# mnlevy1981/MOM6

Measured on AMD Instinct MI355X. Metric: simulated-years/day (SYPD) of the split-RK2 dynamical core + tracer advection + ALE remap, higher is better.
Workload: dtype f64

## Files before the change

### include/mom6hip.h

```cpp
#ifndef MOM6HIP_H
#define MOM6HIP_H

#include <stdint.h>

#ifdef __cplusplus
extern "C" {
#endif

#define MOM6HIP_MEM_HOST   0
#define MOM6HIP_MEM_DEVICE 1

#define MOM6HIP_ADV_PLM    0
#define MOM6HIP_ADV_PPM_H3 1
#define MOM6HIP_ADV_PPM    2

typedef struct mom6hip_grid {
  int32_t isc, iec, jsc, jec;
  int32_t isd, ied, jsd, jed;
  int32_t nk;
  int32_t symmetric;
  int32_t reentrant_x, reentrant_y;
  int32_t first_direction;
  int32_t tripolar_n;
  double Angstrom_H;
// ... 338 lines not shown
#define MOM6HIP_EOS_WRIGHT_REDUCED 5

typedef struct mom6hip_eos {
  int32_t form;
  int32_t reserved;
  double Rho_T0_S0, dRho_dT, dRho_dS;
} mom6hip_eos_t;

typedef struct mom6hip_pressureforce_cs {
  double Rho0;
  double GFS_scale;
  double Z_ref;
  int32_t reconstruct;
  int32_t Recon_Scheme;
  int32_t boundary_extrap;
  int32_t useMassWghtInterp;
  int32_t use_ALE;
  int32_t nkmb;
  double P_Ref;
  const double *Rlay;
  const double *g_prime;
} mom6hip_pressureforce_cs_t;

int mom6hip_pressureforce_fv_bouss(mom6hip_ctx_t *ctx, const mom6hip_pressureforce_cs_t *cs, const mom6hip_eos_t *eos,
                                   const double *h, const double *T, const double *S, const double *p_atm,
                                   double *PFu, double *PFv, double *pbce, double *eta, int32_t memspace);
int mom6hip_pgf_face_launches(mom6hip_ctx_t *ctx, uint64_t *counts);

int mom6hip_pressureforce_fv_nonbouss(mom6hip_ctx_t *ctx, const mom6hip_pressureforce_cs_t *cs, const mom6hip_eos_t *eos,
                                      const double *h, const double *T, const double *S, const double *p_atm, double H_to_RZ,
                                      double *PFu, double *PFv, double *pbce, double *eta, int32_t memspace);

int mom6hip_calculate_density(mom6hip_ctx_t *ctx, const mom6hip_eos_t *eos, const double *T, const double *S,
                              const double *pressure, double *rho, int64_t n, int32_t use_rho_ref, double rho_ref,
                              int32_t memspace);


#define MOM6HIP_BT_HARMONIC     1
#define MOM6HIP_BT_ARITHMETIC   2
#define MOM6HIP_BT_HYBRID       3
#define MOM6HIP_BT_FROM_BT_CONT 4

typedef struct mom6hip_barotropic_cs {
  double dtbt;
  double dtbt_max;
  double dtbt_fraction;
  double bebt;
  double dt_bt_filter;
  double vel_underflow;
  double G_extra;
  double BT_Coriolis_scale;
  double Z_ref;
  double maxCFL_BT_cont;
  double reserved0[6];
  int32_t Sadourny;
  int32_t linearized_BT_PV;
  int32_t strong_drag;
  int32_t visc_rem_u_uh0;
  int32_t adjust_BT_cont;
  int32_t use_wide_halos;
  int32_t hvel_scheme;
  int32_t nstep_last;
  int32_t unsupported[12];
  int32_t bound_BT_corr;
  int32_t BT_project_velocity;
  int32_t Nonlinear_continuity;
  int32_t Nonlin_cont_update_period;
  double *frhatu, *frhatv;
  double *eta_cor;
  double *IDatu, *IDatv;
  double *ubtav, *vbtav;
  double *q_D;
  double *D_u_Cor, *D_v_Cor;
  void *reserved2[6];
} mom6hip_barotropic_cs_t;

int mom6hip_barotropic_init(mom6hip_ctx_t *ctx, mom6hip_barotropic_cs_t *cs, int32_t memspace);

int mom6hip_btcalc(mom6hip_ctx_t *ctx, mom6hip_barotropic_cs_t *cs, const double *h, const double *h_u,
                   const double *h_v, int32_t may_use_default, int32_t memspace);
int mom6hip_btcalc_obc(mom6hip_ctx_t *ctx, mom6hip_barotropic_cs_t *cs, const double *h, const double *h_u, const double *h_v,
                       int32_t may_use_default, const struct mom6hip_obc *obc, int32_t memspace);

int mom6hip_bt_mass_source(mom6hip_ctx_t *ctx, mom6hip_barotropic_cs_t *cs, const double *h, const double *eta,
                           int32_t set_cor, int32_t memspace);

int mom6hip_set_dtbt_eta(mom6hip_ctx_t *ctx, mom6hip_barotropic_cs_t *cs, const double *eta, const double *pbce,
                         const mom6hip_bt_cont_t *BT_cont, double gtot_est, double SSH_add, int32_t memspace);
int mom6hip_set_dtbt(mom6hip_ctx_t *ctx, mom6hip_barotropic_cs_t *cs, const double *pbce,
                     const mom6hip_bt_cont_t *BT_cont, double gtot_est, double SSH_add, int32_t memspace);

int mom6hip_bt_graph_stats(mom6hip_ctx_t *ctx, int64_t *captures, int64_t *launches);
int mom6hip_bt_graph_nodes(mom6hip_ctx_t *ctx, int64_t *nodes);

int mom6hip_btstep(mom6hip_ctx_t *ctx, mom6hip_barotropic_cs_t *cs, const double *U_in, const double *V_in,
                   const double *eta_in, double dt, const double *bc_accel_u, const double *bc_accel_v,
                   const double *taux, const double *tauy, double RZ_to_H, const double *pbce,
                   const double *eta_PF_in, const double *U_Cor, const double *V_Cor, double *accel_layer_u,
                   double *accel_layer_v, double *eta_out, double *uhbtav, double *vhbtav,
                   const double *visc_rem_u, const double *visc_rem_v, const mom6hip_bt_cont_t *BT_cont,
                   const double *eta_PF_start, const double *taux_bot, const double *tauy_bot, const double *uh0,
                   const double *vh0, const double *u_uh0, const double *v_vh0, double *etaav, int32_t memspace);
int mom6hip_btstep_obc(mom6hip_ctx_t *ctx, mom6hip_barotropic_cs_t *cs, const double *U_in, const double *V_in, const double *eta_in,
                       double dt, const double *bc_accel_u, const double *bc_accel_v, const double *taux, const double *tauy,
                       double RZ_to_H, const double *pbce, const double *eta_PF_in, const double *U_Cor, const double *V_Cor,
                       double *accel_layer_u, double *accel_layer_v, double *eta_out, double *uhbtav, double *vhbtav,
                       const double *visc_rem_u, const double *visc_rem_v, const mom6hip_bt_cont_t *BT_cont, const double *eta_PF_start,
                       const double *taux_bot, const double *tauy_bot, const double *uh0, const double *vh0, const double *u_uh0,
                       const double *v_vh0, double *etaav, const struct mom6hip_obc *obc, int32_t memspace);


typedef struct mom6hip_vertvisc_cs {
  double Hmix;
  double Hmix_stress;
  double Kvml_invZ2;
  double Kv;
  double Hbbl;
  double Kv_extra_bbl;
  double harm_BL_val;
  double maxvel;
  double CFL_trunc;
  double vel_underflow;
  double H_to_RZ;
  double vonKar;
  int32_t dynamic_viscous_ML;
  int32_t nkml;
  double reserved0[3];
  int32_t bottomdraglaw;
  int32_t harmonic_visc;
  int32_t direct_stress;
  int32_t CFL_based_trunc;
  int32_t answer_date;
  int32_t unsupported[7];
  int64_t ntrunc;
  double *a_u, *a_v, *h_u, *h_v;
  void *reserved1[4];
} mom6hip_vertvisc_cs_t;

typedef struct mom6hip_vertvisc_type {
  const double *Kv_bbl_u, *Kv_bbl_v;
  const double *bbl_thick_u, *bbl_thick_v;
  const double *Ray_u, *Ray_v;
  const double *Kv_shear;
  const double *Kv_shear_Bu;
  const double *nkml_visc_u, *nkml_visc_v;
  const double *ustar;
  const void *reserved[1];
} mom6hip_vertvisc_type_t;

int mom6hip_vertvisc_coef(mom6hip_ctx_t *ctx, mom6hip_vertvisc_cs_t *cs, const double *u, const double *v, const double *h,
                          const double *dz, const mom6hip_vertvisc_type_t *visc, double dt, int32_t memspace);

int mom6hip_vertvisc(mom6hip_ctx_t *ctx, mom6hip_vertvisc_cs_t *cs, double *u, double *v, const double *h, const double *taux,
                     const double *tauy, const mom6hip_vertvisc_type_t *visc, double dt, double *taux_bot, double *tauy_bot,
                     int32_t memspace);

int mom6hip_vertvisc_coef_obc(mom6hip_ctx_t *ctx, mom6hip_vertvisc_cs_t *cs, const double *u, const double *v, const double *h,
                              const double *dz, const mom6hip_vertvisc_type_t *visc, double dt, const struct mom6hip_obc *obc,
                              int32_t memspace);
int mom6hip_vertvisc_obc(mom6hip_ctx_t *ctx, mom6hip_vertvisc_cs_t *cs, double *u, double *v, const double *h, const double *taux,
                         const double *tauy, const mom6hip_vertvisc_type_t *visc, double dt, double *taux_bot, double *tauy_bot,
                         const struct mom6hip_obc *obc, int32_t memspace);

int mom6hip_vertvisc_and_remnant(mom6hip_ctx_t *ctx, mom6hip_vertvisc_cs_t *cs, double *u, double *v, const double *h,
                                 const double *taux, const double *tauy, const mom6hip_vertvisc_type_t *visc, double dt,
                                 double *taux_bot, double *tauy_bot, double *visc_rem_u, double *visc_rem_v, int32_t memspace);
// ... 310 lines not shown
```

### mom6_amd/_lib.py

```python
import ctypes as C
import os

from . import _abi

_HERE = os.path.dirname(os.path.abspath(__file__))
LIB_PATH = os.environ.get("MOM6HIP_LIB_PATH") or os.path.join(_HERE, "libmom6hip.so")
_LIB = None
_dp = C.POINTER(C.c_double)

EXPORTS = (
    "mom6hip_init", "mom6hip_last_error", "mom6hip_grid_create", "mom6hip_grid_destroy",
    "mom6hip_sync", "mom6hip_malloc", "mom6hip_free", "mom6hip_sync_to_device",
    "mom6hip_sync_to_host", "mom6hip_halo_update", "mom6hip_advect_tracer", "mom6hip_set_timing",
    "mom6hip_advect_get_timing", "mom6hip_ale_remap_tracers", "mom6hip_ale_plm_edge_values", "mom6hip_coradcalc", "mom6hip_continuity", "mom6hip_pressureforce_fv_bouss", "mom6hip_pressureforce_fv_nonbouss", "mom6hip_pgf_face_launches", "mom6hip_calculate_density", "mom6hip_set_domain_callbacks",
    "mom6hip_barotropic_init", "mom6hip_btcalc", "mom6hip_bt_mass_source", "mom6hip_set_dtbt", "mom6hip_memset_zero", "mom6hip_transfer_stats", "mom6hip_debug_poison_passes", "mom6hip_tracer_hordiff_varmix", "mom6hip_tracer_hordiff_neutral", "mom6hip_tracer_hordiff_epipycnal", "mom6hip_continuity_obc", "mom6hip_coradcalc_obc", "mom6hip_vertvisc_coef_obc", "mom6hip_update_segment_tracer_reservoirs", "mom6hip_advect_tracer_obc", "mom6hip_btstep_obc", "mom6hip_horizontal_viscosity_obc", "mom6hip_set_viscous_bbl_obc", "mom6hip_btcalc_obc", "mom6hip_vertvisc_obc", "mom6hip_radiation_open_bdry_conds", "mom6hip_open_boundary_zero_normal_flow", "mom6hip_overlap_stats", "mom6hip_thickness_diffuse", "mom6hip_mixedlayer_restrat", "mom6hip_mixedlayer_restrat_mu", "mom6hip_start_group_pass", "mom6hip_complete_group_pass", "mom6hip_set_dtbt_eta", "mom6hip_btstep",
    "mom6hip_dyn_split_rk2_init", "mom6hip_step_dyn_split_rk2", "mom6hip_dyn_split_rk2b_init", "mom6hip_step_dyn_split_rk2b",
    "mom6hip_ale_regrid", "mom6hip_ale_remap_set_h_vel", "mom6hip_ale_remap_set_h_vel_via_dz", "mom6hip_ale_remap_velocities", "mom6hip_halo_pack", "mom6hip_set_min_callback", "mom6hip_kernel_timing", "mom6hip_set_callback_stream_ordered", "mom6hip_bt_graph_stats", "mom6hip_bt_graph_nodes",
    "mom6hip_vertvisc_coef", "mom6hip_vertvisc", "mom6hip_vertvisc_remnant", "mom6hip_vertvisc_ntrunc", "mom6hip_vertvisc_and_remnant", "mom6hip_vertvisc_step",
    "mom6hip_hor_visc_init", "mom6hip_horizontal_viscosity", "mom6hip_set_viscous_bbl", "mom6hip_set_viscous_ml",
    "mom6hip_chksum", "mom6hip_reproducing_sum", "mom6hip_write_energy_sums", "mom6hip_depth_list_create", "mom6hip_write_energy_ape", "mom6hip_host_register", "mom6hip_host_unregister", "mom6hip_stage_to_host",
    "mom6hip_stage_query", "mom6hip_stage_wait", "mom6hip_stream_bandwidth", "mom6hip_graph_node_floor", "mom6hip_tracer_hordiff", "mom6hip_tracer_hordiff_hbd", "mom6hip_rccl_get_unique_id", "mom6hip_domain_init_rccl", "mom6hip_domain_exchange_timing",
)


class Mom6HipError(RuntimeError):
    pass


def lib():
    global _LIB
    if _LIB is None:
        if not os.path.exists(LIB_PATH):
            raise Mom6HipError(
                f"{LIB_PATH} not found: build it with `python -c 'import __graft_entry__ as g; g.build()'` "
                "(make -C mom6_amd/csrc). mom6_amd has no CPU fallback.")
        import importlib.util
        if importlib.util.find_spec("torch") is not None:
            import torch
        L = C.CDLL(LIB_PATH)
        L.mom6hip_last_error.restype = C.c_char_p
        L.mom6hip_init.argtypes = [C.c_int]
        L.mom6hip_grid_create.argtypes = [C.POINTER(_abi.GridStruct), C.c_void_p, C.POINTER(C.c_void_p)]
        L.mom6hip_grid_destroy.argtypes = [C.c_void_p]
        L.mom6hip_sync.argtypes = [C.c_void_p]
        L.mom6hip_malloc.argtypes = [C.POINTER(C.c_void_p), C.c_uint64]
        L.mom6hip_free.argtypes = [C.c_void_p]
        L.mom6hip_sync_to_device.argtypes = [C.c_void_p, C.c_void_p, C.c_void_p, C.c_uint64]
        L.mom6hip_sync_to_host.argtypes = [C.c_void_p, C.c_void_p, C.c_void_p, C.c_uint64]
        L.mom6hip_halo_update.argtypes = [C.c_void_p, C.POINTER(C.c_void_p), C.POINTER(C.c_int32),
                                          C.POINTER(C.c_int32), C.c_int32]
        L.mom6hip_advect_tracer.argtypes = [
            C.c_void_p, C.c_void_p, C.c_void_p, C.c_void_p, C.c_double,
            C.POINTER(_abi.TracerAdvectCS), C.POINTER(C.c_void_p), _dp, C.c_int32, C.c_int32,
            C.c_void_p, C.c_int32, C.c_int32, C.c_void_p, C.c_void_p, C.c_int32,
            C.POINTER(_abi.AdvectStats)]
        L.mom6hip_set_timing.argtypes = [C.c_void_p, C.c_int32]
        L.mom6hip_advect_get_timing.argtypes = [C.c_void_p, C.POINTER(_abi.AdvectTiming)]
        L.mom6hip_ale_remap_tracers.argtypes = [C.c_void_p, C.POINTER(_abi.RemappingCS), C.c_void_p, C.c_void_p,
                                                C.POINTER(C.c_void_p), _dp, C.c_int32, C.c_int32]
        L.mom6hip_coradcalc.argtypes = [C.c_void_p, C.POINTER(_abi.CoriolisAdvCS)] + [C.c_void_p] * 7 + [C.c_int32]
        L.mom6hip_continuity.argtypes = ([C.c_void_p, C.POINTER(_abi.ContinuityCS)] + [C.c_void_p] * 6 + [C.c_double]
                                         + [C.c_void_p] * 6 + [C.POINTER(_abi.BTCont)] + [C.c_void_p] * 2 + [C.c_int32])
        L.mom6hip_pressureforce_fv_bouss.argtypes = ([C.c_void_p, C.POINTER(_abi.PressureForceCS), C.POINTER(_abi.EOS)]
                                                     + [C.c_void_p] * 8 + [C.c_int32])
        L.mom6hip_pressureforce_fv_nonbouss.argtypes = ([C.c_void_p, C.POINTER(_abi.PressureForceCS), C.POINTER(_abi.EOS)]
                                                        + [C.c_void_p] * 4 + [C.c_double] + [C.c_void_p] * 4 + [C.c_int32])
        L.mom6hip_calculate_density.argtypes = ([C.c_void_p, C.POINTER(_abi.EOS)] + [C.c_void_p] * 4
                                                + [C.c_int64, C.c_int32, C.c_double, C.c_int32])
        L.mom6hip_set_domain_callbacks.argtypes = [C.c_void_p, C.c_void_p, C.c_void_p, C.c_void_p]
        L.mom6hip_kernel_timing.argtypes = [C.c_void_p, C.c_int32, C.POINTER(C.c_double), C.POINTER(C.c_int64)]
        L.mom6hip_bt_graph_stats.argtypes = [C.c_void_p, C.POINTER(C.c_int64), C.POINTER(C.c_int64)]
        L.mom6hip_set_callback_stream_ordered.argtypes = [C.c_void_p, C.c_int32]
        L.mom6hip_set_min_callback.argtypes = [C.c_void_p, C.c_void_p, C.c_void_p]
        L.mom6hip_halo_pack.argtypes = [C.c_void_p, C.POINTER(C.c_void_p), C.POINTER(C.c_int32), C.POINTER(C.c_int32),
                                        C.POINTER(C.c_int32), C.c_int32, C.c_int32, C.c_int32, C.c_void_p, C.c_int32,
                                        C.POINTER(C.c_int64)]
        for n in ("grid", "tracer_advect_cs", "advect_stats", "advect_timing"):
            getattr(L, f"mom6hip_abi_sizeof_{n}").restype = C.c_uint64
        L.mom6hip_abi_offsetof_grid_mask2dT.restype = C.c_uint64
        _LIB = L
    return _LIB


def check(rc, what):
    if rc != 0:
        msg = lib().mom6hip_last_error().decode("utf-8", "replace")
        raise Mom6HipError(f"{what}: {msg} (rc={rc})")
```

### mom6_amd/barotropic.py

```python
from __future__ import annotations

import ctypes as C

import numpy as np
import torch

from . import _abi
from ._lib import Mom6HipError, check, lib
from .continuity import BT_cont_type
from .tracer_advect import DeviceGrid, _ptr_space

_DEFAULTS = dict(dtbt_fraction=0.98, bebt=0.1, dt_bt_filter=-0.25, vel_underflow=0.0, G_extra=0.0, BT_Coriolis_scale=1.0,
                 Z_ref=0.0, Sadourny=True, linearized_BT_PV=True, strong_drag=False, visc_rem_u_uh0=False,
                 adjust_BT_cont=False, use_wide_halos=True)
_PARAM_NAMES = {"BEBT": "bebt", "DT_BT_FILTER": "dt_bt_filter", "VEL_UNDERFLOW": "vel_underflow", "G_BT_EXTRA": "G_extra",
                "BT_CORIOLIS_SCALE": "BT_Coriolis_scale", "REFERENCE_HEIGHT": "Z_ref", "SADOURNY": "Sadourny",
                "LINEARIZED_BT_CORIOLIS": "linearized_BT_PV", "BT_STRONG_DRAG": "strong_drag",
                "BT_USE_VISC_REM_U_UH0": "visc_rem_u_uh0", "ADJUST_BT_CONT": "adjust_BT_cont",
                "BT_USE_WIDE_HALOS": "use_wide_halos"}


class barotropic_CS:

    def __init__(self, G, device="cuda", DTBT=-0.98, BT_THICK_SCHEME=None, USE_BT_CONT_TYPE=True, **params):
        g = G.grid if isinstance(G, DeviceGrid) else G
        d = dict(_DEFAULTS)
        unsupported = [0] * 12
        bound = bool(params.pop("BOUND_BT_CORRECTION", False))
        cont_bounds = bool(params.pop("BT_CONT_CORR_BOUNDS", True))
        maxcfl = float(params.pop("MAXCFL_BT_CONT", 0.25))
        project = bool(params.pop("BT_PROJECT_VELOCITY", False))
        nonlin = bool(params.pop("NONLINEAR_BT_CONTINUITY", False))
        nonlin_period = int(params.pop("NONLIN_BT_CONT_UPDATE_PERIOD", 1))
        if bound and not (USE_BT_CONT_TYPE and cont_bounds):
            unsupported[3] = 1
        for k, v in params.items():
            if k in _PARAM_NAMES:
                d[_PARAM_NAMES[k]] = v
            elif k in d:
                d[k] = v
            elif k in _abi.BT_UNSUPPORTED:
                unsupported[_abi.BT_UNSUPPORTED.index(k)] = int(bool(v))
            else:
                raise Mom6HipError(f"barotropic_init: unknown parameter {k}")
        st = _abi.BarotropicCS()
        for k, v in d.items():
            setattr(st, k, float(v) if isinstance(getattr(st, k), float) else int(bool(v)))
        if BT_THICK_SCHEME is None:
            BT_THICK_SCHEME = "FROM_BT_CONT" if USE_BT_CONT_TYPE else "HYBRID"
        if BT_THICK_SCHEME == "FROM_BT_CONT" and not USE_BT_CONT_TYPE:
            raise Mom6HipError("barotropic_init: BT_THICK_SCHEME FROM_BT_CONT can only be used if USE_BT_CONT_TYPE is defined.")
        st.hvel_scheme = _abi.BT_THICK_SCHEMES[BT_THICK_SCHEME]
        st.bound_BT_corr, st.maxCFL_BT_cont = int(bound), maxcfl
        st.BT_project_velocity = int(project)
        st.Nonlinear_continuity, st.Nonlin_cont_update_period = int(nonlin), nonlin_period
        for q in range(12):
            st.unsupported[q] = unsupported[q]
        self.dtbt_input = float(DTBT)
        st.dtbt_fraction = 0.98 if DTBT >= 0.0 else -float(DTBT)
        st.dtbt = float(DTBT) if DTBT > 0.0 else 0.0
        self.grid, self.device, self.st = g, device, st
        self.arrays = {}
        for n, pos, nd in _abi.BT_CS_ARRAYS:
            shp = g.shape3(pos) if nd == 3 else g.shape2(pos)
            a = np.zeros(shp) if device == "cpu" else torch.zeros(shp, dtype=torch.float64, device=device)
            self.arrays[n] = a
            setattr(st, n, _ptr_space(a)[0])
        self.space = _ptr_space(self.arrays["frhatu"])[1]
        self.module_is_initialized = False

    def __getattr__(self, n):
        a = self.__dict__.get("arrays", {})
        if n in a:
            return a[n]
        st = self.__dict__.get("st")
        if st is not None and hasattr(st, n):
            return getattr(st, n)
        raise AttributeError(n)


def _P(spaces, a):
    if a is None:
        return None
    p, s = _ptr_space(a)
    spaces.add(s)
    return C.c_void_p(p)


def _one_space(spaces, CS, who):
    spaces.add(CS.space)
    if len(spaces) != 1:
        raise Mom6HipError(f"{who}: all fields and the control structure must be in the same memory space")
    return spaces.pop()


def _setup():
    L = lib()
    if not getattr(L, "_bt_ready", False):
        cs = C.POINTER(_abi.BarotropicCS)
        L.mom6hip_barotropic_init.argtypes = [C.c_void_p, cs, C.c_int32]
        L.mom6hip_btcalc.argtypes = [C.c_void_p, cs, C.c_void_p, C.c_void_p, C.c_void_p, C.c_int32, C.c_int32]
        L.mom6hip_btcalc_obc.argtypes = [C.c_void_p, cs, C.c_void_p, C.c_void_p, C.c_void_p, C.c_int32, C.POINTER(_abi.Obc), C.c_int32]
        L.mom6hip_bt_mass_source.argtypes = [C.c_void_p, cs, C.c_void_p, C.c_void_p, C.c_int32, C.c_int32]
        L.mom6hip_set_dtbt.argtypes = [C.c_void_p, cs, C.c_void_p, C.POINTER(_abi.BTCont), C.c_double, C.c_double, C.c_int32]
        L.mom6hip_set_dtbt_eta.argtypes = [C.c_void_p, cs, C.c_void_p, C.c_void_p, C.POINTER(_abi.BTCont), C.c_double, C.c_double, C.c_int32]
        L.mom6hip_btstep.argtypes = ([C.c_void_p, cs] + [C.c_void_p] * 3 + [C.c_double] + [C.c_void_p] * 4 + [C.c_double]
                                     + [C.c_void_p] * 11 + [C.POINTER(_abi.BTCont)] + [C.c_void_p] * 8 + [C.c_int32])
        L.mom6hip_btstep_obc.argtypes = ([C.c_void_p, cs] + [C.c_void_p] * 3 + [C.c_double] + [C.c_void_p] * 4 + [C.c_double]
                                         + [C.c_void_p] * 11 + [C.POINTER(_abi.BTCont)] + [C.c_void_p] * 8 + [C.POINTER(_abi.Obc), C.c_int32])
        L._bt_ready = True
    return L


def barotropic_init(G: DeviceGrid, device="cuda", gtot_estimate=None, SSH_extra=None, **params) -> barotropic_CS:
    CS = barotropic_CS(G, device=device, **params)
    L = _setup()
    check(L.mom6hip_barotropic_init(G.handle, C.byref(CS.st), CS.space), "barotropic_init")
    CS.module_is_initialized = True
    g = CS.grid
    if gtot_estimate is None:
        gtot_estimate = g.H_to_Z * g.g_Earth
    if SSH_extra is None:
        SSH_extra = min(10.0, 0.05 * float(np.max(g.bathyT)))
    dtbt_in = CS.dtbt_input
    set_dtbt(G, CS, gtot_est=gtot_estimate, SSH_add=SSH_extra)
    if dtbt_in > 0.0:
        CS.st.dtbt = dtbt_in
    return CS


def btcalc(h, G: DeviceGrid, CS: barotropic_CS, h_u=None, h_v=None, may_use_default=False, OBC=None):
    if not CS.module_is_initialized:
        raise Mom6HipError("btcalc: Module MOM_barotropic must be initialized before it is used.")
    sp = set()
    args = [_P(sp, h), _P(sp, h_u), _P(sp, h_v)]
    if OBC is not None:
        obc = OBC.struct(lambda a: (0, None))
        check(_setup().mom6hip_btcalc_obc(G.handle, C.byref(CS.st), *args, int(bool(may_use_default)), C.byref(obc),
                                          _one_space(sp, CS, "btcalc")), "btcalc")
        return
    check(_setup().mom6hip_btcalc(G.handle, C.byref(CS.st), *args, int(bool(may_use_default)), _one_space(sp, CS, "btcalc")), "btcalc")


def bt_mass_source(h, eta, set_cor, G: DeviceGrid, CS: barotropic_CS):
    if not CS.module_is_initialized:
        raise Mom6HipError("bt_mass_source: Module MOM_barotropic must be initialized before it is used.")
    sp = set()
    args = [_P(sp, h), _P(sp, eta)]
    check(_setup().mom6hip_bt_mass_source(G.handle, C.byref(CS.st), *args, int(bool(set_cor)), _one_space(sp, CS, "bt_mass_source")),
          "bt_mass_source")


def set_dtbt(G: DeviceGrid, CS: barotropic_CS, eta=None, pbce=None, BT_cont: BT_cont_type | None = None, gtot_est=None,
             SSH_add=0.0):
    if not CS.module_is_initialized:
        raise Mom6HipError("set_dtbt: Module MOM_barotropic must be initialized before it is used.")
    if pbce is None and gtot_est is None:
        raise Mom6HipError("set_dtbt: Either pbce or gtot_est must be present.")
    sp = set()
    p = _P(sp, pbce)
    pe = _P(sp, eta)
    bt = None if BT_cont is None else BT_cont.struct(sp)
    check(_setup().mom6hip_set_dtbt_eta(G.handle, C.byref(CS.st), pe, p, None if bt is None else C.byref(bt),
                                    0.0 if gtot_est is None else float(gtot_est), float(SSH_add), _one_space(sp, CS, "set_dtbt")),
          "set_dtbt")
    return CS.st.dtbt_max


def btstep(U_in, V_in, eta_in, dt, bc_accel_u, bc_accel_v, forces, pbce, eta_PF_in, U_Cor, V_Cor, accel_layer_u,
           accel_layer_v, eta_out, uhbtav, vhbtav, G: DeviceGrid, CS: barotropic_CS, visc_rem_u, visc_rem_v, SpV_avg=None,
           ADp=None, OBC=None, BT_cont: BT_cont_type | None = None, eta_PF_start=None, taux_bot=None, tauy_bot=None, uh0=None,
           vh0=None, u_uh0=None, v_vh0=None, etaav=None):
    if not CS.module_is_initialized:
        raise Mom6HipError("btstep: Module MOM_barotropic must be initialized before it is used.")
    if (uh0 is not None) and (vh0 is None or u_uh0 is None or v_vh0 is None):
        raise Mom6HipError("btstep: vh0, u_uh0, and v_vh0 must be associated if uh0 is used.")
    g = CS.grid
    taux, tauy = forces
    sp = set()
    P = lambda a: _P(sp, a)
    a1 = [P(U_in), P(V_in), P(eta_in)]
    a2 = [P(bc_accel_u), P(bc_accel_v), P(taux), P(tauy)]
    a3 = [P(x) for x in (pbce, eta_PF_in, U_Cor, V_Cor, accel_layer_u, accel_layer_v, eta_out, uhbtav, vhbtav, visc_rem_u, visc_rem_v)]
    bt = None if BT_cont is None else BT_cont.struct(sp)
    a4 = [P(x) for x in (eta_PF_start, taux_bot, tauy_bot, uh0, vh0, u_uh0, v_vh0, etaav)]
    RZ_to_H = g.Z_to_H / g.Rho0
    space = _one_space(sp, CS, "btstep")
    if OBC is not None:
        from .open_boundary import _seg_to_ptr
        obc = OBC.struct(_seg_to_ptr(space))
        check(_setup().mom6hip_btstep_obc(G.handle, C.byref(CS.st), *a1, float(dt), *a2, float(RZ_to_H), *a3,
                                          None if bt is None else C.byref(bt), *a4, C.byref(obc), space), "btstep")
        return
    check(_setup().mom6hip_btstep(G.handle, C.byref(CS.st), *a1, float(dt), *a2, float(RZ_to_H), *a3,
                                  None if bt is None else C.byref(bt), *a4, space), "btstep")
```

### mom6_amd/csrc/barotropic.hip

```cpp
#include "common.hpp"
#include "cr_math.hpp"

#include <algorithm>
#include <string>
#include <cmath>
#include <cstdlib>
#include <functional>
#include <initializer_list>
#include <utility>

namespace m6 {

}

namespace {

constexpr double SUBROUNDOFF = 1e-30;

using m6::cr::cr_pow;

template <class F> __global__ void __launch_bounds__(256) range2d_kernel(int i0, int i1, int j0, int j1, F f) {
  const int i = i0 + blockIdx.x * 64 + threadIdx.x, j = j0 + blockIdx.y * 4 + threadIdx.y;
  if (i <= i1 && j <= j1) f(i, j);
}
// ... 4 lines not shown
}

struct Btcl { double *FA_EE, *FA_E0, *FA_W0, *FA_WW, *uBT_WW, *uBT_EE, *uh_crvW, *uh_crvE, *uh_WW, *uh_EE; };

__device__ __forceinline__ double find_uhbt(double u, const Btcl &B, long n) {
  if (u == 0.0) return 0.0;
  const double ee = B.uBT_EE[n];
  if (u < ee) return (u - ee) * B.FA_EE[n] + B.uh_EE[n];
  if (u < 0.0) return u * (B.FA_E0[n] + B.uh_crvE[n] * (u * u));
  const double ww = B.uBT_WW[n];
  if (u <= ww) return u * (B.FA_W0[n] + B.uh_crvW[n] * (u * u));
  return (u - ww) * B.FA_WW[n] + B.uh_WW[n];
}

struct Work {
  double *ubt, *bt_rem_u, *BT_force_u, *u_accel_bt, *uhbt, *uhbt0, *uhbtp, *azon, *bzon, *czon, *dzon, *Cor_ref_u,
      *DCor_u, *Datu, *ubt_Cor, *ubt0, *uhbtS, *amer, *bmer, *cmer, *dmer;
  double *vbt, *bt_rem_v, *BT_force_v, *v_accel_bt, *vhbt, *vhbt0, *vhbtp, *Cor_ref_v, *DCor_v, *Datv, *vbt_Cor, *vbt0,
      *vhbtS;
  double *eta, *eta_pred, *eta_sum, *eta_wtd, *eta_PF, *eta_PF_1, *d_eta_PF, *gtot_E, *gtot_W, *gtot_N, *gtot_S,
      *eta_src, *e_anom;
  double *q;
  Btcl BU, BV;
  const int32_t *obc_u, *obc_v;
  double *ob_Cg_u, *ob_dZ_u, *ob_uhbt, *ob_ubt_outer, *ob_SSH_u, *ubt_old, *ubt_first, *ubt_wtd;
  double *ob_Cg_v, *ob_dZ_v, *ob_vhbt, *ob_vbt_outer, *ob_SSH_v, *vbt_old, *vbt_first, *vbt_wtd;
};
enum { OB_SPEC = 1, OB_FLATHER = 2, OB_GRAD = 4, OB_PLUS = 8, OB_MINUS = 16 };

__device__ double uhbt_to_ubt(double uhbt, const Btcl &B, long n) {
  const double tol = 1.0e-10;
  const int max_itt = 20;
  double ubt, ubt_min, ubt_max, uherr_min, uherr_max;
  if (uhbt == 0.0) {
    ubt = 0.0;
  } else if (uhbt < B.uh_EE[n]) {
    ubt = B.uBT_EE[n] + (uhbt - B.uh_EE[n]) / B.FA_EE[n];
  } else if (uhbt < 0.0) {
    ubt_min = B.uBT_EE[n]; uherr_min = B.uh_EE[n] - uhbt;
    ubt_max = 0.0; uherr_max = -uhbt;
    ubt = B.uBT_EE[n] * (uhbt / B.uh_EE[n]);
    for (int itt = 1; itt <= max_itt; itt++) {
      const double uhbt_err = ubt * (B.FA_E0[n] + B.uh_crvE[n] * (ubt * ubt)) - uhbt;
      if (fabs(uhbt_err) < tol * fabs(uhbt)) break;
      if (uhbt_err > 0.0) { ubt_max = ubt; uherr_max = uhbt_err; }
      if (uhbt_err < 0.0) { ubt_min = ubt; uherr_min = uhbt_err; }
      const double derr_du = B.FA_E0[n] + 3.0 * B.uh_crvE[n] * (ubt * ubt);
      if ((uhbt_err >= derr_du * (ubt - ubt_min)) || (-uhbt_err >= derr_du * (ubt_max - ubt)) || (derr_du <= 0.0)) {
        ubt = ubt_max + (ubt_min - ubt_max) * (uherr_max / (uherr_max - uherr_min));
      } else {
        ubt = ubt - uhbt_err / derr_du;
        if (fabs(uhbt_err) < (0.01 * tol) * fabs(ubt_min * derr_du)) break;
      }
    }
  } else if (uhbt <= B.uh_WW[n]) {
    ubt_min = 0.0; uherr_min = -uhbt;
    ubt_max = B.uBT_WW[n]; uherr_max = B.uh_WW[n] - uhbt;
    ubt = B.uBT_WW[n] * (uhbt / B.uh_WW[n]);
    for (int itt = 1; itt <= max_itt; itt++) {
      const double uhbt_err = ubt * (B.FA_W0[n] + B.uh_crvW[n] * (ubt * ubt)) - uhbt;
      if (fabs(uhbt_err) < tol * fabs(uhbt)) break;
      if (uhbt_err > 0.0) { ubt_max = ubt; uherr_max = uhbt_err; }
      if (uhbt_err < 0.0) { ubt_min = ubt; uherr_min = uhbt_err; }
      const double derr_du = B.FA_W0[n] + 3.0 * B.uh_crvW[n] * (ubt * ubt);
      if ((uhbt_err >= derr_du * (ubt - ubt_min)) || (-uhbt_err >= derr_du * (ubt_max - ubt)) || (derr_du <= 0.0)) {
        ubt = ubt_min + (ubt_max - ubt_min) * (-uherr_min / (uherr_max - uherr_min));
      } else {
        ubt = ubt - uhbt_err / derr_du;
        if (fabs(uhbt_err) < (0.01 * tol) * (ubt_max * derr_du)) break;
      }
    }
  } else {
    ubt = B.uBT_WW[n] + (uhbt - B.uh_WW[n]) / B.FA_WW[n];
  }
  return ubt;
}

struct Par {
  double dtbt, Instep, dgeo_de, vel_underflow, trans_wt1, trans_wt2, RZ_to_H;
  int project_velocity;
  int nstep, use_BT_cont, interp_eta_PF, add_uh0, strong_drag, visc_rem_u_uh0, find_etaav, have_bot;
};

template <int DIR>
__global__ void __launch_bounds__(256)
bt_pre_face_kernel(m6::GridDev g, Work w, Par p, const double *__restrict__ frhat, const double *__restrict__ visc_rem,
                   const double *__restrict__ vel_Cor, const double *__restrict__ pbce, const double *__restrict__ uh0,
                   const double *__restrict__ u_uh0, const double *__restrict__ vel_in, const double *__restrict__ bc_accel,
                   const double *__restrict__ tau, const double *__restrict__ tau_bot, const double *__restrict__ IDat) {
  const int i = (DIR ? g.isc : g.isc - 1) + blockIdx.x * 64 + threadIdx.x;
  const int j = (DIR ? g.jsc - 1 : g.jsc) + blockIdx.y * 4 + threadIdx.y;
  if (i > g.iec || j > g.jec) return;
  const long f2 = DIR ? g.v2(i, j) : g.u2(i, j);
  const long fstr = DIR ? (long)g.nih * (g.njh + 1) : (long)(g.nih + 1) * g.njh;
  const long hm = g.h2(i, j), hp = DIR ? g.h2(i, j + 1) : g.h2(i + 1, j), hstr = (long)g.nih * g.njh;
  const double mask = DIR ? g.mask2dCv[f2] : g.mask2dCu[f2];

  double vel_cor = 0.0, gt_m = 0.0, gt_p = 0.0, uhS = 0.0, u0 = 0.0, ub = 0.0, av_rem = 0.0, force;
  if (mask > 0.0) {
    force = tau[f2] * p.RZ_to_H * IDat[f2] * visc_rem[f2];
    if (p.have_bot) force = force - tau_bot[f2] * p.RZ_to_H * IDat[f2];
  } else {
    force = 0.0;
  }
  for (int k = 0; k < g.nk; k++) {
    const long f3 = f2 + fstr * k;
    const double fr = frhat[f3], vr_in = visc_rem[f3];
    double vr = m6::min2(vr_in, 1.);
    vr = m6::max2(vr, 1. - 0.5 * p.Instep / (vr + SUBROUNDOFF));
    vr = m6::max2(vr, 0.);
    const double wt = fr * vr;
    vel_cor = vel_cor + wt * vel_Cor[f3];
    gt_m = gt_m + pbce[hm + hstr * k] * wt;
    gt_p = gt_p + pbce[hp + hstr * k] * wt;
    if (p.add_uh0) {
      uhS = uhS + uh0[f3];
      u0 = u0 + (p.visc_rem_u_uh0 ? wt : fr) * u_uh0[f3];
    }
    ub = ub + wt * vel_in[f3];
    force = force + wt * bc_accel[f3];
    av_rem = av_rem + fr * vr_in;
  }
  if (fabs(ub) < p.vel_underflow) ub = 0.0;
  double rem;
  if (p.strong_drag) {
    rem = mask * ((p.nstep * av_rem) / (1.0 + (p.nstep - 1) * av_rem));
  } else {
    rem = 0.0;
    if (mask * av_rem > 0.0) rem = mask * cr_pow(av_rem, p.Instep);
  }
  if (DIR == 0) {
    w.ubt_Cor[f2] = vel_cor; w.gtot_E[hm] = gt_m; w.gtot_W[hp] = gt_p; w.uhbtS[f2] = uhS; w.ubt0[f2] = u0;
    w.ubt[f2] = ub; w.BT_force_u[f2] = force; w.bt_rem_u[f2] = rem;
  } else {
    w.vbt_Cor[f2] = vel_cor; w.gtot_N[hm] = gt_m; w.gtot_S[hp] = gt_p; w.vhbtS[f2] = uhS; w.vbt0[f2] = u0;
    w.vbt[f2] = ub; w.BT_force_v[f2] = force; w.bt_rem_v[f2] = rem;
  }
}

template <int DIR, int NKMAX>
__global__ void __launch_bounds__(256) __attribute__((amdgpu_waves_per_eu(3, 8)))
btcalc_given_kernel(m6::GridDev g, const double *__restrict__ hw, double *__restrict__ fr, double h_neglect) {
  const int i = (DIR ? g.isc : g.isc - 1) + blockIdx.x * 64 + threadIdx.x;
  const int j = (DIR ? g.jsc - 1 : g.jsc) + blockIdx.y * 4 + threadIdx.y;
  if (i > g.iec || j > g.jec) return;
  const long f2 = DIR ? g.v2(i, j) : g.u2(i, j);
  const long fstr = DIR ? (long)g.nih * (g.njh + 1) : (long)(g.nih + 1) * g.njh;
  const double mask = DIR ? g.mask2dCv[f2] : g.mask2dCu[f2];
  const int nz = g.nk;
  double v[NKMAX];
  const double *__restrict__ src = hw + f2;
#pragma unroll
  for (int k = 0; k < NKMAX; k++) { v[k] = (k < nz) ? *src : 0.0; src += fstr; }
  double tot = v[0];
#pragma unroll
  for (int k = 1; k < NKMAX; k++) if (k < nz) tot = tot + v[k];
  const double Ihat = mask / (tot + h_neglect);
  double *__restrict__ dst = fr + f2;
#pragma unroll
  for (int k = 0; k < NKMAX; k++) { if (k < nz) *dst = v[k] * Ihat; dst += fstr; }
}

template <int DIR>
__global__ void __launch_bounds__(256)
bt_accel_layer_kernel(m6::GridDev g, Work w, const double *__restrict__ pbce, double *__restrict__ accel, double accel_underflow) {
  const int i = (DIR ? g.isc : g.isc - 1) + blockIdx.x * 64 + threadIdx.x;
  const int j = (DIR ? g.jsc - 1 : g.jsc) + blockIdx.y * 4 + threadIdx.y;
  if (i > g.iec || j > g.jec) return;
  const long f2 = DIR ? g.v2(i, j) : g.u2(i, j);
  const long fstr = DIR ? (long)g.nih * (g.njh + 1) : (long)(g.nih + 1) * g.njh;
  const long hm = g.h2(i, j), hp = DIR ? g.h2(i, j + 1) : g.h2(i + 1, j), hstr = (long)g.nih * g.njh;
  const double abt = DIR ? w.v_accel_bt[f2] : w.u_accel_bt[f2];
  const double gp = DIR ? w.gtot_S[hp] : w.gtot_W[hp], gm = DIR ? w.gtot_N[hm] : w.gtot_E[hm];
  const double ep = w.e_anom[hp], em = w.e_anom[hm];
  const double Id = DIR ? g.IdyCv[f2] : g.IdxCu[f2];
  for (int k = 0; k < g.nk; k++) {
    double a = (abt - ((pbce[hp + hstr * k] - gp) * ep - (pbce[hm + hstr * k] - gm) * em) * Id);
    if (fabs(a) < accel_underflow) a = 0.0;
    accel[f2 + fstr * k] = a;
  }
}

__global__ void __launch_bounds__(256)
bt_eta_pred_kernel(m6::GridDev g, Work w, Par p, int i0, int i1, int j0, int j1, double wt_accel2) {
  const int i = i0 + blockIdx.x * 64 + threadIdx.x, j = j0 + blockIdx.y * 4 + threadIdx.y;
  if (i > i1 || j > j1) return;
  const long n = g.h2(i, j);
  double ep;
  if (p.project_velocity) {
    ep = w.eta[n];
  } else {
    ep = (w.eta[n] + w.eta_src[n]) + (p.dtbt * g.IareaT[n]) *
        ((w.uhbtp[g.u2(i - 1, j)] - w.uhbtp[g.u2(i, j)]) + (w.vhbtp[g.v2(i, j - 1)] - w.vhbtp[g.v2(i, j)]));
    w.eta_pred[n] = ep;
  }
  if (p.find_etaav && i >= g.isc && i <= g.iec && j >= g.jsc && j <= g.jec) w.eta_sum[n] = w.eta_sum[n] + wt_accel2 * ep;
}

__global__ void __launch_bounds__(256)
bt_eta_kernel(m6::GridDev g, Work w, Par p, int i0, int i1, int j0, int j1, double wt_eta) {
  const int i = i0 + blockIdx.x * 64 + threadIdx.x, j = j0 + blockIdx.y * 4 + threadIdx.y;
  if (i > i1 || j > j1) return;
  const long n = g.h2(i, j);
  const double e = (w.eta[n] + w.eta_src[n]) + (p.dtbt * g.IareaT[n]) *
      ((w.uhbt[g.u2(i - 1, j)] - w.uhbt[g.u2(i, j)]) + (w.vhbt[g.v2(i, j - 1)] - w.vhbt[g.v2(i, j)]));
  w.eta[n] = e;
  w.eta_wtd[n] = w.eta_wtd[n] + e * wt_eta;
}

__device__ __forceinline__ double eta_pf_at(const Work &w, const Par &p, long n, double wt_end) {
  return p.interp_eta_PF ? (w.eta_PF_1[n] + wt_end * w.d_eta_PF[n]) : w.eta_PF[n];
}

__global__ void __launch_bounds__(256)
bt_vbt_kernel(m6::GridDev g, Work w, Par p, int i0, int i1, int j0, int j1, double wt_accel, double wt_trans, double wt_end,
              double *__restrict__ vbt_sum, double *__restrict__ vhbt_sum) {
  const int i = i0 + blockIdx.x * 64 + threadIdx.x, J = j0 + blockIdx.y * 4 + threadIdx.y;
  if (i > i1 || J > j1) return;
  const int j = J;
  const long n = g.v2(i, J);
  if (w.obc_v && w.obc_v[n]) return;
  const double Cor_v = -1.0 * ((w.amer[g.u2(i - 1, j)] * w.ubt[g.u2(i - 1, j)] + w.cmer[g.u2(i, j + 1)] * w.ubt[g.u2(i, j + 1)]) +
                               (w.bmer[g.u2(i, j)] * w.ubt[g.u2(i, j)] + w.dmer[g.u2(i - 1, j + 1)] * w.ubt[g.u2(i - 1, j + 1)])) -
                       w.Cor_ref_v[n];
  const long hs = g.h2(i, j), hn = g.h2(i, j + 1);
  const double *epb = p.project_velocity ? w.eta : w.eta_pred;
  const double PFv = ((epb[hs] - eta_pf_at(w, p, hs, wt_end)) * w.gtot_N[hs] -
                      (epb[hn] - eta_pf_at(w, p, hn, wt_end)) * w.gtot_S[hn]) * p.dgeo_de * g.IdyCv[n];
  const double vel_prev = w.vbt[n];
  double vb = w.bt_rem_v[n] * (vel_prev + p.dtbt * ((w.BT_force_v[n] + Cor_v) + PFv));
  if (fabs(vb) < p.vel_underflow) vb = 0.0;
  const double vtrans = p.trans_wt1 * vb + p.trans_wt2 * vel_prev;
  w.vbt[n] = vb;
  w.v_accel_bt[n] = w.v_accel_bt[n] + wt_accel * (Cor_v + PFv);
  const double vh0 = w.vhbt0[n];
  double vh, vhp;
  if (p.use_BT_cont) { vh = find_uhbt(vtrans, w.BV, n) + vh0; vhp = find_uhbt(vb, w.BV, n) + vh0; }
  else { const double D = w.Datv[n]; vh = D * vtrans + vh0; vhp = D * vb + vh0; }
  w.vhbt[n] = vh; w.vhbtp[n] = vhp;
  if (i >= g.isc && i <= g.iec && J >= g.jsc - 1 && J <= g.jec) {
    vbt_sum[n] = vbt_sum[n] + wt_trans * vtrans;
    vhbt_sum[n] = vhbt_sum[n] + wt_trans * vh;
  }
}

__global__ void __launch_bounds__(256)
bt_ubt_kernel(m6::GridDev g, Work w, Par p, int i0, int i1, int j0, int j1, double wt_accel, double wt_trans, double wt_end,
              double *__restrict__ ubt_sum, double *__restrict__ uhbt_sum) {
  const int I = i0 + blockIdx.x * 64 + threadIdx.x, j = j0 + blockIdx.y * 4 + threadIdx.y;
  if (I > i1 || j > j1) return;
  const int i = I;
  const long n = g.u2(I, j);
  if (w.obc_u && w.obc_u[n]) return;
  const double Cor_u = ((w.azon[n] * w.vbt[g.v2(i + 1, j)] + w.czon[n] * w.vbt[g.v2(i, j - 1)]) +
                        (w.bzon[n] * w.vbt[g.v2(i, j)] + w.dzon[n] * w.vbt[g.v2(i + 1, j - 1)])) - w.Cor_ref_u[n];
  const long hw = g.h2(i, j), he = g.h2(i + 1, j);
  const double *epb = p.project_velocity ? w.eta : w.eta_pred;
  const double PFu = ((epb[hw] - eta_pf_at(w, p, hw, wt_end)) * w.gtot_E[hw] -
                      (epb[he] - eta_pf_at(w, p, he, wt_end)) * w.gtot_W[he]) * p.dgeo_de * g.IdxCu[n];
  const double vel_prev = w.ubt[n];
  double ub = w.bt_rem_u[n] * (vel_prev + p.dtbt * ((w.BT_force_u[n] + Cor_u) + PFu));
  if (fabs(ub) < p.vel_underflow) ub = 0.0;
// ... 188 lines not shown
        vel_trans = (1.0 - bebt) * vel_prev + bebt * vb;
      } else { vb = 0.0; vel_trans = 0.0; }
    } else {
      vb = xbt[f + df];
      vel_trans = vb;
    }
  }
  xbt[f] = vb;
  double xh = xhbt[f];
  if (!(code & OB_SPEC)) {
    xh = (p.use_BT_cont ? find_uhbt(vel_trans, B, f) : Dat * vel_trans) + xhbt0;
    xhbt[f] = xh;
  }
  xhbtp[f] = (p.use_BT_cont ? find_uhbt(vb, B, f) : Dat * vb) + xhbt0;
  const bool own = DIR ? (i >= g.isc && i <= g.iec && j >= g.jsc - 1 && j <= g.jec) : (i >= g.isc - 1 && i <= g.iec && j >= g.jsc && j <= g.jec);
  if (own) {
    xbt_sum[f] = xbt_sum[f] + wt_trans * vel_trans;
    xhbt_sum[f] = xhbt_sum[f] + wt_trans * xh;
    xwtd[f] = xwtd[f] + wt_vel * vb;
  }
}

__global__ void __launch_bounds__(256)
bt_dtbt_kernel(m6::GridDev g, const double *__restrict__ pbce, const double *__restrict__ frhatu, const double *__restrict__ frhatv,
               const double *__restrict__ Datu, const double *__restrict__ Datv, double gtot_est, double bebt, double cor_scale,
               unsigned long long *__restrict__ result) {
  const int i = g.isc + blockIdx.x * 64 + threadIdx.x, j = g.jsc + blockIdx.y * 4 + threadIdx.y;
  double cand = 1.0e38;
  if (i <= g.iec && j <= g.jec) {
    const long n = g.h2(i, j);
    double gE = 0.0, gW = 0.0, gN = 0.0, gS = 0.0;
    if (pbce) {
      const long hstr = (long)g.nih * g.njh, ustr = (long)(g.nih + 1) * g.njh, vstr = (long)g.nih * (g.njh + 1);
      for (int k = 0; k < g.nk; k++) {
        const double pb = pbce[n + hstr * k];
        gE = gE + pb * frhatu[g.u2(i, j) + ustr * k];
        gW = gW + pb * frhatu[g.u2(i - 1, j) + ustr * k];
        gN = gN + pb * frhatv[g.v2(i, j) + vstr * k];
        gS = gS + pb * frhatv[g.v2(i, j - 1) + vstr * k];
      }
    } else {
      gE = gW = gN = gS = gtot_est;
    }
    const double f00 = g.CoriolisBu[g.q2(i, j)], f11 = g.CoriolisBu[g.q2(i - 1, j - 1)], f10 = g.CoriolisBu[g.q2(i - 1, j)],
                 f01 = g.CoriolisBu[g.q2(i, j - 1)];
    const double Idt_max2 = 0.5 * (1.0 + 2.0 * bebt) * (g.IareaT[n] *
        ((gE * Datu[g.u2(i, j)] * g.IdxCu[g.u2(i, j)] + gW * Datu[g.u2(i - 1, j)] * g.IdxCu[g.u2(i - 1, j)]) +
         (gN * Datv[g.v2(i, j)] * g.IdyCv[g.v2(i, j)] + gS * Datv[g.v2(i, j - 1)] * g.IdyCv[g.v2(i, j - 1)])) +
        ((f00 * f00 + f11 * f11) + (f10 * f10 + f01 * f01)) * (cor_scale * cor_scale));
    if (Idt_max2 * 1.0e38 > 1.0) cand = 1.0 / Idt_max2;
  }
  __shared__ unsigned long long smin;
  if (threadIdx.x == 0 && threadIdx.y == 0) smin = 0x7FF0000000000000ull;
  __syncthreads();
  atomicMin(&smin, (unsigned long long)__double_as_longlong(cand));
  __syncthreads();
  if (threadIdx.x == 0 && threadIdx.y == 0) atomicMin(result, smin);
}

int check_cs(const mom6hip_barotropic_cs_t *cs, const char *who) {
  M6_REQUIRE(cs != nullptr, "%s: null control structure", who);
  static const char *names[12] = {"INTEGRAL_BT_CONTINUITY", "(free slot)", "NONLINEAR_BT_CONTINUITY", "BOUND_BT_CORRECTION without BT_CONT_CORR_BOUNDS / USE_BT_CONT_TYPE",
                                  "GRADUAL_BT_ICS", "BT_NONLIN_STRESS", "DYNAMIC_SURFACE_PRESSURE", "BT_LINEAR_WAVE_DRAG",
                                  "CLIP_BT_VELOCITY", "CALCULATE_SAL", "BT_USE_OLD_CORIOLIS_BRACKET_BUG",
                                  "BAROTROPIC_ANSWER_DATE < 20190101"};
  for (int q = 0; q < 12; q++)
    M6_REQUIRE(cs->unsupported[q] == 0, "%s: %s is not provided by libmom6hip", who, names[q]);
  return 0;
}

struct Sizes { size_t h2, u2, v2, q2, h3, u3, v3; };
Sizes sizes_of(const m6::GridDev &g) {
  Sizes s;
  s.h2 = sizeof(double) * (size_t)g.nih * g.njh; s.u2 = sizeof(double) * (size_t)(g.nih + 1) * g.njh;
  s.v2 = sizeof(double) * (size_t)g.nih * (g.njh + 1); s.q2 = sizeof(double) * (size_t)(g.nih + 1) * (g.njh + 1);
  s.h3 = s.h2 * g.nk; s.u3 = s.u2 * g.nk; s.v3 = s.v2 * g.nk;
  return s;
}

struct CsDev { double *frhatu, *frhatv, *eta_cor, *IDatu, *IDatv, *ubtav, *vbtav, *q_D, *D_u_Cor, *D_v_Cor; };

dim3 grid2d(int i0, int i1, int j0, int j1) { return dim3((i1 - i0 + 64) / 64, (j1 - j0 + 4) / 4); }

}

extern "C" {

int mom6hip_barotropic_init(mom6hip_ctx_t *ctx, mom6hip_barotropic_cs_t *cs, int32_t memspace) {
  M6_REQUIRE(ctx != nullptr, "barotropic_init: null context");
  if (int rc = check_cs(cs, "barotropic_init")) return rc;
  const m6::GridDev g = ctx->g;
  M6_REQUIRE(g.bathyT && g.areaT && g.mask2dT && g.mask2dCu && g.mask2dCv && g.CoriolisBu,
             "barotropic_init: bathyT, areaT, mask2dT, mask2dCu, mask2dCv and CoriolisBu are needed");
  M6_REQUIRE(cs->frhatu && cs->frhatv && cs->eta_cor && cs->IDatu && cs->IDatv && cs->ubtav && cs->vbtav,
             "barotropic_init: the control structure's state arrays must be allocated");
  M6_REQUIRE(!cs->linearized_BT_PV || (cs->q_D && cs->D_u_Cor && cs->D_v_Cor), "barotropic_init: q_D, D_u_Cor, D_v_Cor needed");
  const Sizes sz = sizes_of(g);
  m6::Stager st(ctx, memspace);
  CsDev d;
  d.frhatu = st.out(cs->frhatu, sz.u3); d.frhatv = st.out(cs->frhatv, sz.v3); d.eta_cor = st.out(cs->eta_cor, sz.h2);
  d.IDatu = st.out(cs->IDatu, sz.u2); d.IDatv = st.out(cs->IDatv, sz.v2); d.ubtav = st.out(cs->ubtav, sz.u2);
  d.vbtav = st.out(cs->vbtav, sz.v2);
  const bool lin = cs->linearized_BT_PV != 0;
  d.q_D = lin ? st.out(cs->q_D, sz.q2) : nullptr; d.D_u_Cor = lin ? st.out(cs->D_u_Cor, sz.u2) : nullptr;
  d.D_v_Cor = lin ? st.out(cs->D_v_Cor, sz.v2) : nullptr;
  M6_REQUIRE(!st.failed(), "barotropic_init: staging failed");
  hipStream_t s = ctx->stream;
  M6_HIP(hipMemsetAsync(d.frhatu, 0, sz.u3, s)); M6_HIP(hipMemsetAsync(d.frhatv, 0, sz.v3, s));
  M6_HIP(hipMemsetAsync(d.eta_cor, 0, sz.h2, s)); M6_HIP(hipMemsetAsync(d.IDatu, 0, sz.u2, s));
  M6_HIP(hipMemsetAsync(d.IDatv, 0, sz.v2, s)); M6_HIP(hipMemsetAsync(d.ubtav, 0, sz.u2, s));
  M6_HIP(hipMemsetAsync(d.vbtav, 0, sz.v2, s));
  const double Z_to_H = g.Z_to_H, Mean_SL = cs->Z_ref, scale = cs->BT_Coriolis_scale, hsub = g.H_subroundoff;
  if (cs->linearized_BT_PV) {
    M6_HIP(hipMemsetAsync(d.q_D, 0, sz.q2, s)); M6_HIP(hipMemsetAsync(d.D_u_Cor, 0, sz.u2, s));
    M6_HIP(hipMemsetAsync(d.D_v_Cor, 0, sz.v2, s));
    launch2d(s, g.isc - 1, g.iec, g.jsc, g.jec, [=] __device__(int I, int j) {
      d.D_u_Cor[g.u2(I, j)] = 0.5 * (m6::max2(Mean_SL + g.bathyT[g.h2(I + 1, j)], 0.0) + m6::max2(Mean_SL + g.bathyT[g.h2(I, j)], 0.0)) * Z_to_H;
    });
    launch2d(s, g.isc, g.iec, g.jsc - 1, g.jec, [=] __device__(int i, int J) {
      d.D_v_Cor[g.v2(i, J)] = 0.5 * (m6::max2(Mean_SL + g.bathyT[g.h2(i, J + 1)], 0.0) + m6::max2(Mean_SL + g.bathyT[g.h2(i, J)], 0.0)) * Z_to_H;
    });
    launch2d(s, g.isc - 1, g.iec, g.jsc - 1, g.jec, [=] __device__(int i, int j) {
      auto BT = [&](int a, int b) { return g.bathyT[g.h2(a, b)]; };
      auto AT = [&](int a, int b) { return g.areaT[g.h2(a, b)]; };
      auto MT = [&](int a, int b) { return g.mask2dT[g.h2(a, b)]; };
      double qv = 0.;
      if (MT(i, j) + MT(i, j + 1) + MT(i + 1, j) + MT(i + 1, j + 1) > 0.) {
        qv = 0.25 * (scale * g.CoriolisBu[g.q2(i, j)]) * ((AT(i, j) + AT(i + 1, j + 1)) + (AT(i + 1, j) + AT(i, j + 1))) /
             (Z_to_H * m6::max2(((AT(i, j) * m6::max2(Mean_SL + BT(i, j), 0.0) + AT(i + 1, j + 1) * m6::max2(Mean_SL + BT(i + 1, j + 1), 0.0)) +
                                 (AT(i + 1, j) * m6::max2(Mean_SL + BT(i + 1, j), 0.0) + AT(i, j + 1) * m6::max2(Mean_SL + BT(i, j + 1), 0.0))),
                                hsub));
      }
      d.q_D[g.q2(i, j)] = qv;
    });
    double *f[3] = {d.q_D, d.D_u_Cor, d.D_v_Cor};
    const int32_t pos[3] = {MOM6HIP_POS_Q, MOM6HIP_POS_U | MOM6HIP_PASS_SCALAR_PAIR, MOM6HIP_POS_V | MOM6HIP_PASS_SCALAR_PAIR},
                  nk[3] = {1, 1, 1};
    if (int rc = m6::group_pass(ctx, f, pos, nk, 3)) return rc;
  }
  launch2d(s, g.isc - 1, g.iec, g.jsc, g.jec, [=] __device__(int I, int j) {
    const double m = g.mask2dCu[g.u2(I, j)];
    d.IDatu[g.u2(I, j)] = (m > 0.) ? m * 2.0 / (Z_to_H * ((g.bathyT[g.h2(I + 1, j)] + g.bathyT[g.h2(I, j)]) + 2.0 * Mean_SL)) : 0.;
  });
  launch2d(s, g.isc, g.iec, g.jsc - 1, g.jec, [=] __device__(int i, int J) {
    const double m = g.mask2dCv[g.v2(i, J)];
    d.IDatv[g.v2(i, J)] = (m > 0.) ? m * 2.0 / (Z_to_H * ((g.bathyT[g.h2(i, J + 1)] + g.bathyT[g.h2(i, J)]) + 2.0 * Mean_SL)) : 0.;
  });
  M6_HIP(hipGetLastError());
  return st.finish();
}

int mom6hip_btcalc(mom6hip_ctx_t *ctx, mom6hip_barotropic_cs_t *cs, const double *h, const double *h_u, const double *h_v,
                   int32_t may_use_default, int32_t memspace) {
  return mom6hip_btcalc_obc(ctx, cs, h, h_u, h_v, may_use_default, nullptr, memspace);
}

int mom6hip_btcalc_obc(mom6hip_ctx_t *ctx, mom6hip_barotropic_cs_t *cs, const double *h, const double *h_u, const double *h_v,
                       int32_t may_use_default, const mom6hip_obc_t *obc, int32_t memspace) {
  M6_REQUIRE(ctx != nullptr && cs != nullptr && h != nullptr, "btcalc: null argument");
  const m6::GridDev g = ctx->g;
  const int sch = cs->hvel_scheme;
  int use_default = 0;
  const bool given = h_u && h_v;
  if (!(given || sch == MOM6HIP_BT_HARMONIC || sch == MOM6HIP_BT_HYBRID || sch == MOM6HIP_BT_ARITHMETIC)) {
    M6_REQUIRE(may_use_default, "btcalc: Inconsistent settings of optional arguments and hvel_scheme.");
    use_default = 1;
  }
  const Sizes sz = sizes_of(g);
  m6::Stager st(ctx, memspace);
  const double *dh = st.in(h, sz.h3), *dhu = given ? st.in(h_u, sz.u3) : nullptr, *dhv = given ? st.in(h_v, sz.v3) : nullptr;
  double *fru = st.inout(cs->frhatu, sz.u3), *frv = st.inout(cs->frhatv, sz.v3);
  M6_REQUIRE(!st.failed(), "btcalc: staging failed");
  const double h_neglect = g.H_subroundoff, Z_to_H = g.Z_to_H;
  const int hybrid = (sch == MOM6HIP_BT_HYBRID || use_default), arith = (sch == MOM6HIP_BT_ARITHMETIC);
  const int32_t *side_d[2] = {nullptr, nullptr};
  if (obc && obc->OBC_pe && m6::obc_side_maps(ctx, st, obc, &side_d[0], &side_d[1], "btcalc")) return 1;
  for (int dir = 0; dir < 2; dir++) {
    const double *hw = dir ? dhv : dhu;
    const int32_t *side = side_d[dir];
    double *fr = dir ? frv : fru;
    const long fstr = dir ? (long)g.nih * (g.njh + 1) : (long)(g.nih + 1) * g.njh, hstr = (long)g.nih * g.njh;
    if (hw && !side && g.nk <= 76) {
      const dim3 grid = grid2d(dir ? g.isc : g.isc - 1, g.iec, dir ? g.jsc - 1 : g.jsc, g.jec), block(64, 4);
      if (g.nk <= 32) {
        if (dir) hipLaunchKernelGGL((btcalc_given_kernel<1, 32>), grid, block, 0, ctx->stream, g, hw, fr, h_neglect);
        else hipLaunchKernelGGL((btcalc_given_kernel<0, 32>), grid, block, 0, ctx->stream, g, hw, fr, h_neglect);
      } else {
        if (dir) hipLaunchKernelGGL((btcalc_given_kernel<1, 76>), grid, block, 0, ctx->stream, g, hw, fr, h_neglect);
        else hipLaunchKernelGGL((btcalc_given_kernel<0, 76>), grid, block, 0, ctx->stream, g, hw, fr, h_neglect);
      }
      continue;
    }
    launch2d(ctx->stream, dir ? g.isc : g.isc - 1, g.iec, dir ? g.jsc - 1 : g.jsc, g.jec, [=] __device__(int i, int j) {
      const long f2 = dir ? g.v2(i, j) : g.u2(i, j);
      const long hm = g.h2(i, j), hp = dir ? g.h2(i, j + 1) : g.h2(i + 1, j);
      const double mask = dir ? g.mask2dCv[f2] : g.mask2dCu[f2];
      const int nz = g.nk;
      double tot;
      if (side && side[f2]) {
        const long hc = side[f2] < 0 ? hm : hp;
        tot = dh[hc];
        for (int k = 1; k < nz; k++) tot = tot + dh[hc + hstr * k];
        const double Ihtot = mask / (tot + h_neglect);
        for (int k = 0; k < nz; k++) fr[f2 + fstr * k] = dh[hc + hstr * k] * Ihtot;
        return;
      }
      if (hw) {
        tot = hw[f2];
        for (int k = 1; k < nz; k++) tot = tot + hw[f2 + fstr * k];
        const double Ihat = mask / (tot + h_neglect);
        for (int k = 0; k < nz; k++) fr[f2 + fstr * k] = hw[f2 + fstr * k] * Ihat;
        return;
      }
      if (arith) {
        tot = 0.0;
        for (int k = 0; k < nz; k++) {
          const double v = 0.5 * (dh[hp + hstr * k] + dh[hm + hstr * k]);
          fr[f2 + fstr * k] = v;
          tot = (k == 0) ? v : tot + v;
        }
      } else if (hybrid) {
        const double bp = g.bathyT[hp], bm = g.bathyT[hm];
        double e_below = -0.5 * Z_to_H * (bp + bm);
        const double D_shallow = -Z_to_H * m6::min2(bp, bm);
        tot = 0.0;
        for (int k = nz - 1; k >= 0; k--) {
          const double a = dh[hp + hstr * k], b = dh[hm + hstr * k];
          const double e_here = e_below + 0.5 * (a + b);
          const double h_arith = 0.5 * (a + b);
          double v;
          if (e_below >= D_shallow) {
            v = h_arith;
          } else {
            const double h_harm = (a * b) / (h_arith + h_neglect);
            if (e_here <= D_shallow) {
              v = h_harm;
            } else {
              const double wt_arith = (e_here - D_shallow) / (h_arith + h_neglect);
              v = wt_arith * h_arith + (1.0 - wt_arith) * h_harm;
            }
          }
          fr[f2 + fstr * k] = v;
          tot = tot + v;
          e_below = e_here;
        }
      } else {
        tot = 0.0;
        for (int k = 0; k < nz; k++) {
          const double a = dh[hp + hstr * k], b = dh[hm + hstr * k];
          const double v = 2.0 * (a * b) / ((a + b) + h_neglect);
          fr[f2 + fstr * k] = v;
          tot = (k == 0) ? v : tot + v;
        }
      }
      const double Ihat = mask / (tot + h_neglect);
      for (int k = 0; k < nz; k++) fr[f2 + fstr * k] = fr[f2 + fstr * k] * Ihat;
    });
  }
  M6_HIP(hipGetLastError());
  return st.finish();
}

int mom6hip_bt_mass_source(mom6hip_ctx_t *ctx, mom6hip_barotropic_cs_t *cs, const double *h, const double *eta, int32_t set_cor,
                           int32_t memspace) {
  M6_REQUIRE(ctx != nullptr && cs != nullptr && h != nullptr && eta != nullptr, "bt_mass_source: null argument");
  const m6::GridDev g = ctx->g;
  const Sizes sz = sizes_of(g);
  m6::Stager st(ctx, memspace);
  const double *dh = st.in(h, sz.h3), *de = st.in(eta, sz.h2);
  double *cor = st.inout(cs->eta_cor, sz.h2);
  M6_REQUIRE(!st.failed(), "bt_mass_source: staging failed");
  const long hstr = (long)g.nih * g.njh;
  const double Z_to_H = g.Z_to_H;
  launch2d(ctx->stream, g.isc, g.iec, g.jsc, g.jec, [=] __device__(int i, int j) {
    const long n = g.h2(i, j);
    double eta_h = dh[n] - g.bathyT[n] * Z_to_H;
    for (int k = 1; k < g.nk; k++) eta_h = eta_h + dh[n + hstr * k];
    const double d_eta = eta_h - de[n];
    cor[n] = set_cor ? d_eta : cor[n] + d_eta;
  });
  M6_HIP(hipGetLastError());
  return st.finish();
}

int mom6hip_set_dtbt(mom6hip_ctx_t *ctx, mom6hip_barotropic_cs_t *cs, const double *pbce, const mom6hip_bt_cont_t *BT_cont,
                     double gtot_est, double SSH_add, int32_t memspace) {
  return mom6hip_set_dtbt_eta(ctx, cs, nullptr, pbce, BT_cont, gtot_est, SSH_add, memspace);
}

int mom6hip_set_dtbt_eta(mom6hip_ctx_t *ctx, mom6hip_barotropic_cs_t *cs, const double *eta, const double *pbce,
                         const mom6hip_bt_cont_t *BT_cont, double gtot_est, double SSH_add, int32_t memspace) {
  M6_REQUIRE(ctx != nullptr, "set_dtbt: null context");
  if (int rc = check_cs(cs, "set_dtbt")) return rc;
  const m6::GridDev g = ctx->g;
  const Sizes sz = sizes_of(g);
  m6::Stager st(ctx, memspace);
  const double *dp = pbce ? st.in(pbce, sz.h3) : nullptr;
  const double *deta = (eta && !BT_cont && cs->Nonlinear_continuity) ? st.in(eta, sz.h2) : nullptr;
  const double *fru = pbce ? st.in((const double *)cs->frhatu, sz.u3) : nullptr, *frv = pbce ? st.in((const double *)cs->frhatv, sz.v3) : nullptr;
  double *Datu = (double *)st.scratch(sz.u2), *Datv = (double *)st.scratch(sz.v2);
  unsigned long long *res = (unsigned long long *)st.scratch(sizeof(unsigned long long));
  const double *FA[8] = {};
  if (BT_cont) {
    const double *src[8] = {BT_cont->FA_u_EE, BT_cont->FA_u_E0, BT_cont->FA_u_W0, BT_cont->FA_u_WW,
                            BT_cont->FA_v_NN, BT_cont->FA_v_N0, BT_cont->FA_v_S0, BT_cont->FA_v_SS};
    for (int q = 0; q < 8; q++) { M6_REQUIRE(src[q], "set_dtbt: BT_cont is incomplete"); FA[q] = st.in(src[q], q < 4 ? sz.u2 : sz.v2); }
  }
  M6_REQUIRE(!st.failed() && Datu && Datv && res, "set_dtbt: staging failed");
  hipStream_t s = ctx->stream;
  M6_HIP(hipMemsetAsync(Datu, 0, sz.u2, s)); M6_HIP(hipMemsetAsync(Datv, 0, sz.v2, s));
  const unsigned long long inf_bits = 0x7FF0000000000000ull;
  M6_HIP(hipMemcpyAsync(res, &inf_bits, sizeof(inf_bits), hipMemcpyHostToDevice, s));
  if (BT_cont) {
    const double *a0 = FA[0], *a1 = FA[1], *a2 = FA[2], *a3 = FA[3], *b0 = FA[4], *b1 = FA[5], *b2 = FA[6], *b3 = FA[7];
    launch2d(s, g.isc - 1, g.iec, g.jsc, g.jec, [=] __device__(int I, int j) {
      const long n = g.u2(I, j);
      Datu[n] = m6::max2(m6::max2(m6::max2(a0[n], a1[n]), a2[n]), a3[n]);
    });
    launch2d(s, g.isc, g.iec, g.jsc - 1, g.jec, [=] __device__(int i, int J) {
      const long n = g.v2(i, J);
      Datv[n] = m6::max2(m6::max2(m6::max2(b0[n], b1[n]), b2[n]), b3[n]);
    });
  } else if (deta) {
    const double Z_to_H = g.Z_to_H;
    launch2d(s, g.isc - 1, g.iec, g.jsc, g.jec, [=] __device__(int I, int j) {
      const double H1 = g.bathyT[g.h2(I, j)] * Z_to_H + deta[g.h2(I, j)], H2 = g.bathyT[g.h2(I + 1, j)] * Z_to_H + deta[g.h2(I + 1, j)];
      double D = 0.0;
      if ((H1 > 0.0) && (H2 > 0.0)) D = g.dy_Cu[g.u2(I, j)] * (2.0 * H1 * H2) / (H1 + H2);
      Datu[g.u2(I, j)] = D;
    });
    launch2d(s, g.isc, g.iec, g.jsc - 1, g.jec, [=] __device__(int i, int J) {
      const double H1 = g.bathyT[g.h2(i, J)] * Z_to_H + deta[g.h2(i, J)], H2 = g.bathyT[g.h2(i, J + 1)] * Z_to_H + deta[g.h2(i, J + 1)];
      double D = 0.0;
      if ((H1 > 0.0) && (H2 > 0.0)) D = g.dx_Cv[g.v2(i, J)] * (2.0 * H1 * H2) / (H1 + H2);
      Datv[g.v2(i, J)] = D;
    });
  } else {
    const double Z_to_H = g.Z_to_H, add = cs->Z_ref + SSH_add;
    launch2d(s, g.isc - 1, g.iec, g.jsc, g.jec, [=] __device__(int I, int j) {
      Datu[g.u2(I, j)] = g.dy_Cu[g.u2(I, j)] * Z_to_H * m6::max2(m6::max2(g.bathyT[g.h2(I + 1, j)], g.bathyT[g.h2(I, j)]) + add, 0.0);
    });
    launch2d(s, g.isc, g.iec, g.jsc - 1, g.jec, [=] __device__(int i, int J) {
      Datv[g.v2(i, J)] = g.dx_Cv[g.v2(i, J)] * Z_to_H * m6::max2(m6::max2(g.bathyT[g.h2(i, J + 1)], g.bathyT[g.h2(i, J)]) + add, 0.0);
    });
  }
  hipLaunchKernelGGL(bt_dtbt_kernel, grid2d(g.isc, g.iec, g.jsc, g.jec), dim3(64, 4), 0, s, g, dp, fru, frv, Datu, Datv, gtot_est,
                     cs->bebt, cs->BT_Coriolis_scale, res);
  M6_HIP(hipGetLastError());
  unsigned long long bits = 0;
  if (m6::multi_tile(ctx)) {
    if (int rc = m6::min_across_PEs_dev_u64(ctx, (unsigned long long *)res, 1, &bits)) return rc;
  } else {
    M6_HIP(hipMemcpyAsync(&bits, res, sizeof(bits), hipMemcpyDeviceToHost, s));
    M6_HIP(hipStreamSynchronize(s));
  }
  double min_max_dt2;
  memcpy(&min_max_dt2, &bits, sizeof(double));
  if (!(min_max_dt2 < 1.0e38)) min_max_dt2 = 1.0e38;
  const double dgeo_de = 1.0 + (cs->G_extra > 0.0 ? cs->G_extra : 0.0);
  const double dtbt_max = sqrt(min_max_dt2 / dgeo_de);
  cs->dtbt = cs->dtbt_fraction * dtbt_max;
  cs->dtbt_max = dtbt_max;
  return st.finish();
}

int mom6hip_btstep(mom6hip_ctx_t *ctx, mom6hip_barotropic_cs_t *cs, const double *U_in, const double *V_in, const double *eta_in,
                   double dt, const double *bc_accel_u, const double *bc_accel_v, const double *taux, const double *tauy,
                   double RZ_to_H, const double *pbce, const double *eta_PF_in, const double *U_Cor, const double *V_Cor,
                   double *accel_layer_u, double *accel_layer_v, double *eta_out, double *uhbtav, double *vhbtav,
                   const double *visc_rem_u, const double *visc_rem_v, const mom6hip_bt_cont_t *BT_cont, const double *eta_PF_start,
                   const double *taux_bot, const double *tauy_bot, const double *uh0, const double *vh0, const double *u_uh0,
                   const double *v_vh0, double *etaav, int32_t memspace) {
  return mom6hip_btstep_obc(ctx, cs, U_in, V_in, eta_in, dt, bc_accel_u, bc_accel_v, taux, tauy, RZ_to_H, pbce, eta_PF_in, U_Cor, V_Cor,
                            accel_layer_u, accel_layer_v, eta_out, uhbtav, vhbtav, visc_rem_u, visc_rem_v, BT_cont, eta_PF_start, taux_bot,
                            tauy_bot, uh0, vh0, u_uh0, v_vh0, etaav, nullptr, memspace);
}

int mom6hip_btstep_obc(mom6hip_ctx_t *ctx, mom6hip_barotropic_cs_t *cs, const double *U_in, const double *V_in, const double *eta_in,
                   double dt, const double *bc_accel_u, const double *bc_accel_v, const double *taux, const double *tauy,
                   double RZ_to_H, const double *pbce, const double *eta_PF_in, const double *U_Cor, const double *V_Cor,
                   double *accel_layer_u, double *accel_layer_v, double *eta_out, double *uhbtav, double *vhbtav,
                   const double *visc_rem_u, const double *visc_rem_v, const mom6hip_bt_cont_t *BT_cont, const double *eta_PF_start,
                   const double *taux_bot, const double *tauy_bot, const double *uh0, const double *vh0, const double *u_uh0,
                   const double *v_vh0, double *etaav, const mom6hip_obc_t *obc, int32_t memspace) {
  M6_REQUIRE(ctx != nullptr, "btstep: null context");
  if (int rc = check_cs(cs, "btstep")) return rc;
  M6_REQUIRE(U_in && V_in && eta_in && bc_accel_u && bc_accel_v && taux && tauy && pbce && eta_PF_in && U_Cor && V_Cor &&
                 accel_layer_u && accel_layer_v && eta_out && uhbtav && vhbtav && visc_rem_u && visc_rem_v,
             "btstep: a required argument is null");
  M6_REQUIRE((uh0 != nullptr) == (vh0 != nullptr && u_uh0 != nullptr && v_vh0 != nullptr),
             "btstep: vh0, u_uh0, and v_vh0 must be associated if uh0 is used.");
  M6_REQUIRE(cs->dtbt > 0.0 && dt > 0.0, "btstep: dt and CS%%dtbt must be positive (call set_dtbt first)");
  const m6::GridDev g = ctx->g;
  M6_REQUIRE(g.bathyT && g.IareaT && g.areaT && g.IdxCu && g.IdyCv && g.dy_Cu && g.dx_Cv && g.mask2dT && g.mask2dCu &&
                 g.mask2dCv && g.CoriolisBu, "btstep: a metric array it needs was not given to grid_create");
  const int is = g.isc, ie = g.iec, js = g.jsc, je = g.jec;
  const Sizes sz = sizes_of(g);
  const bool use_BT_cont = BT_cont != nullptr, interp = eta_PF_start != nullptr, add_uh0 = uh0 != nullptr;
  const bool find_etaav = etaav != nullptr, have_bot = taux_bot && tauy_bot;
  const bool nonlin_cont = !use_BT_cont && cs->Nonlinear_continuity;
  const bool nonlin_update = nonlin_cont && cs->Nonlin_cont_update_period > 0;
  const int stencil = nonlin_update ? 2 : 1;

  int num_cycles = 1;
  if (cs->use_wide_halos) num_cycles = std::min((is - g.isd) / stencil, (js - g.jsd) / stencil);
  M6_REQUIRE(num_cycles >= 1, "btstep: the grid has no halo");
  const int isvf = is - (num_cycles - 1) * stencil, ievf = ie + (num_cycles - 1) * stencil;
  const int jsvf = js - (num_cycles - 1) * stencil, jevf = je + (num_cycles - 1) * stencil;
  const int nstep = (int)ceil(dt / cs->dtbt - 0.0001);
  M6_REQUIRE(nstep >= 1, "btstep: nstep < 1");
  cs->nstep_last = nstep;

  Par p;
  p.Instep = 1.0 / (double)nstep; p.dtbt = dt * p.Instep; p.dgeo_de = 1.0 + cs->G_extra; p.vel_underflow = cs->vel_underflow;
  p.project_velocity = cs->BT_project_velocity ? 1 : 0;
  p.trans_wt1 = p.project_velocity ? (1.0 + cs->bebt) : cs->bebt; p.trans_wt2 = p.project_velocity ? -cs->bebt : (1.0 - cs->bebt);
  p.RZ_to_H = RZ_to_H; p.nstep = nstep; p.use_BT_cont = use_BT_cont;
  p.interp_eta_PF = interp; p.add_uh0 = add_uh0; p.strong_drag = cs->strong_drag; p.visc_rem_u_uh0 = cs->visc_rem_u_uh0;
  p.find_etaav = find_etaav; p.have_bot = have_bot;
  const double accel_underflow = cs->vel_underflow * (1.0 / dt);

  double dt_filt;
  if (cs->dt_bt_filter >= 0.0) dt_filt = 0.5 * std::max(0.0, std::min(cs->dt_bt_filter, 2.0 * dt));
  else dt_filt = 0.5 * std::max(0.0, dt * std::min(-cs->dt_bt_filter, 2.0));
  const int nfilter = (int)ceil(dt_filt / p.dtbt);
  const int nt = nstep + nfilter;
  M6_REQUIRE(nt > 0, "btstep: number of barotropic step (nstep+nfilter) is 0");
  std::vector<double> wt_vel(nt + 2, 0.0), wt_eta(nt + 2, 0.0), wt_trans(nt + 2, 0.0), wt_accel(nt + 2, 0.0), wt_accel2(nt + 2, 0.0);
  {
    double sum_wt_vel = 0.0, sum_wt_eta = 0.0, sum_wt_accel = 0.0, sum_wt_trans = 0.0;
    for (int n = 1; n <= nt; n++) {
      if ((n == nstep) || (dt_filt - abs(n - nstep) * p.dtbt >= 0.0)) { wt_vel[n] = 1.0; wt_eta[n] = 1.0; }
      else if (p.dtbt + dt_filt - abs(n - nstep) * p.dtbt > 0.0) { wt_vel[n] = 1.0 + (dt_filt / p.dtbt) - abs(n - nstep); wt_eta[n] = wt_vel[n]; }
      else { wt_vel[n] = 0.0; wt_eta[n] = 0.0; }
      sum_wt_vel = sum_wt_vel + wt_vel[n]; sum_wt_eta = sum_wt_eta + wt_eta[n];
    }
    for (int n = nt; n >= 1; n--) {
      wt_trans[n] = wt_trans[n + 1] + wt_eta[n];
      wt_accel[n] = wt_accel[n + 1] + wt_vel[n];
      sum_wt_accel = sum_wt_accel + wt_accel[n]; sum_wt_trans = sum_wt_trans + wt_trans[n];
    }
    const double Iv = 1.0 / sum_wt_vel, Ia = 1.0 / sum_wt_accel, Ie = 1.0 / sum_wt_eta, It = 1.0 / sum_wt_trans;
    for (int n = 1; n <= nt; n++) {
      wt_vel[n] = wt_vel[n] * Iv; wt_accel2[n] = wt_accel[n] * Ia; wt_trans[n] = wt_trans[n] * It;
      wt_accel[n] = wt_accel[n] * Ia; wt_eta[n] = wt_eta[n] * Ie;
    }
  }

  m6::Stager st(ctx, memspace);
  const double *dU = st.in(U_in, sz.u3), *dV = st.in(V_in, sz.v3), *deta_in = st.in(eta_in, sz.h2);
  const double *dbu = st.in(bc_accel_u, sz.u3), *dbv = st.in(bc_accel_v, sz.v3), *dtx = st.in(taux, sz.u2), *dty = st.in(tauy, sz.v2);
  const double *dpb = st.in(pbce, sz.h3), *depf = st.in(eta_PF_in, sz.h2), *dUc = st.in(U_Cor, sz.u3), *dVc = st.in(V_Cor, sz.v3);
  const double *dvru = st.in(visc_rem_u, sz.u3), *dvrv = st.in(visc_rem_v, sz.v3);
  const double *depfs = st.in(eta_PF_start, sz.h2), *dtbx = have_bot ? st.in(taux_bot, sz.u2) : nullptr,
               *dtby = have_bot ? st.in(tauy_bot, sz.v2) : nullptr;
  const double *duh0 = st.in(uh0, sz.u3), *dvh0 = st.in(vh0, sz.v3), *duu0 = st.in(u_uh0, sz.u3), *dvv0 = st.in(v_vh0, sz.v3);
  double *dalu = st.inout(accel_layer_u, sz.u3), *dalv = st.inout(accel_layer_v, sz.v3);
  double *deta_out = st.inout(eta_out, sz.h2);
  double *duhbtav = st.inout(uhbtav, sz.u2), *dvhbtav = st.inout(vhbtav, sz.v2), *detaav = st.inout(etaav, sz.h2);
  CsDev c;
  c.frhatu = st.inout(cs->frhatu, sz.u3); c.frhatv = st.inout(cs->frhatv, sz.v3); c.eta_cor = st.inout(cs->eta_cor, sz.h2);
  c.IDatu = st.inout(cs->IDatu, sz.u2); c.IDatv = st.inout(cs->IDatv, sz.v2);
  c.ubtav = st.inout(cs->ubtav, sz.u2); c.vbtav = st.inout(cs->vbtav, sz.v2);
  c.q_D = cs->linearized_BT_PV ? st.inout(cs->q_D, sz.q2) : nullptr;
  c.D_u_Cor = cs->linearized_BT_PV ? st.inout(cs->D_u_Cor, sz.u2) : nullptr;
  c.D_v_Cor = cs->linearized_BT_PV ? st.inout(cs->D_v_Cor, sz.v2) : nullptr;
  M6_REQUIRE(!cs->linearized_BT_PV || (c.q_D && c.D_u_Cor && c.D_v_Cor), "btstep: q_D, D_u_Cor and D_v_Cor are needed (barotropic_init)");
  const double *bcU[6] = {}, *bcV[6] = {};
  if (use_BT_cont) {
    const double *su[6] = {BT_cont->FA_u_EE, BT_cont->FA_u_E0, BT_cont->FA_u_W0, BT_cont->FA_u_WW, BT_cont->uBT_EE, BT_cont->uBT_WW};
    const double *sv[6] = {BT_cont->FA_v_NN, BT_cont->FA_v_N0, BT_cont->FA_v_S0, BT_cont->FA_v_SS, BT_cont->vBT_NN, BT_cont->vBT_SS};
    for (int q = 0; q < 6; q++) {
      M6_REQUIRE(su[q] && sv[q], "btstep: BT_cont is incomplete");
      bcU[q] = st.in(su[q], sz.u2); bcV[q] = st.in(sv[q], sz.v2);
    }
  }
  const int NU_ARR = 21 + 10, NV_ARR = 13 + 10, NH_ARR = 13;
  const size_t total = NU_ARR * sz.u2 + NV_ARR * sz.v2 + NH_ARR * sz.h2 + sz.q2;
  char *blk = (char *)st.scratch(total);
// ... 144 lines not shown
    launch2d(s, g.isd, g.ied, g.jsd, g.jed, [=] __device__(int i, int j) { w.d_eta_PF[g.h2(i, j)] = depf[g.h2(i, j)] - depfs[g.h2(i, j)]; });
  } else {
    M6_HIP(hipMemcpyAsync(w.eta_PF, depf, sz.h2, hipMemcpyDeviceToDevice, s));
  }

  const int hs = 1 + ievf - ie;
  const bool early_btcl_pass = use_BT_cont && add_uh0 && cs->adjust_BT_cont;
  std::function<void(int)> btcl_derive;
  auto face_areas_eta = [&](hipStream_t fs, int hs) {
    const double Z_to_H = g.Z_to_H;
    launch2d(fs, is - 1 - hs, ie + hs, js - hs, je + hs, [=] __device__(int I, int j) {
      const double H1 = g.bathyT[g.h2(I, j)] * Z_to_H + w.eta[g.h2(I, j)], H2 = g.bathyT[g.h2(I + 1, j)] * Z_to_H + w.eta[g.h2(I + 1, j)];
      double D = 0.0;
      if ((H1 > 0.0) && (H2 > 0.0)) D = g.dy_Cu[g.u2(I, j)] * (2.0 * H1 * H2) / (H1 + H2);
      w.Datu[g.u2(I, j)] = D;
    });
    launch2d(fs, is - hs, ie + hs, js - 1 - hs, je + hs, [=] __device__(int i, int J) {
      const double H1 = g.bathyT[g.h2(i, J)] * Z_to_H + w.eta[g.h2(i, J)], H2 = g.bathyT[g.h2(i, J + 1)] * Z_to_H + w.eta[g.h2(i, J + 1)];
      double D = 0.0;
      if ((H1 > 0.0) && (H2 > 0.0)) D = g.dx_Cv[g.v2(i, J)] * (2.0 * H1 * H2) / (H1 + H2);
      w.Datv[g.v2(i, J)] = D;
    });
  };
  if (use_BT_cont) {
    const Btcl BU = w.BU, BV = w.BV;
    const double *a0 = bcU[0], *a1 = bcU[1], *a2 = bcU[2], *a3 = bcU[3], *a4 = bcU[4], *a5 = bcU[5];
    const double *b0 = bcV[0], *b1 = bcV[1], *b2 = bcV[2], *b3 = bcV[3], *b4 = bcV[4], *b5 = bcV[5];
    launch2d(s, is - 1, ie, js, je, [=] __device__(int I, int j) {
      const long n = g.u2(I, j);
      BU.FA_EE[n] = a0[n]; BU.FA_E0[n] = a1[n]; BU.FA_W0[n] = a2[n]; BU.FA_WW[n] = a3[n]; BU.uBT_EE[n] = a4[n]; BU.uBT_WW[n] = a5[n];
    });
    launch2d(s, is, ie, js - 1, je, [=] __device__(int i, int J) {
      const long n = g.v2(i, J);
      BV.FA_EE[n] = b0[n]; BV.FA_E0[n] = b1[n]; BV.FA_W0[n] = b2[n]; BV.FA_WW[n] = b3[n]; BV.uBT_EE[n] = b4[n]; BV.uBT_WW[n] = b5[n];
    });
    btcl_derive = [=](int hs_) {
      for (int dir = 0; dir < 2; dir++) {
        const Btcl B = dir ? BV : BU;
        launch2d(s, (dir ? is : is - 1) - hs_, ie + hs_, (dir ? js - 1 : js) - hs_, je + hs_, [=] __device__(int i, int j) {
          const long n = dir ? g.v2(i, j) : g.u2(i, j);
          const double C1_3 = 1.0 / 3.0;
          if (g.tripolar_n && j > je) {
            double t = B.FA_EE[n]; B.FA_EE[n] = B.FA_WW[n]; B.FA_WW[n] = t;
            t = B.FA_E0[n]; B.FA_E0[n] = B.FA_W0[n]; B.FA_W0[n] = t;
            t = B.uBT_EE[n]; B.uBT_EE[n] = B.uBT_WW[n]; B.uBT_WW[n] = t;
          }
          const double ee = 1.0 * B.uBT_EE[n], ww = 1.0 * B.uBT_WW[n];
          B.uBT_EE[n] = ee; B.uBT_WW[n] = ww;
          B.uh_EE[n] = ee * (C1_3 * (2.0 * B.FA_E0[n] + B.FA_EE[n]));
          B.uh_WW[n] = ww * (C1_3 * (2.0 * B.FA_W0[n] + B.FA_WW[n]));
          double cw = 0.0, ce = 0.0;
          if (fabs(ww) > 0.0) cw = (C1_3 * (B.FA_WW[n] - B.FA_W0[n])) / (ww * ww);
          if (fabs(ee) > 0.0) ce = (C1_3 * (B.FA_EE[n] - B.FA_E0[n])) / (ee * ee);
          B.uh_crvW[n] = cw; B.uh_crvE[n] = ce;
        });
      }
    };
    if (early_btcl_pass) {
      if (int rc = pass({{BU.uBT_EE, PU}, {BV.uBT_EE, PV}, {BU.uBT_WW, PU}, {BV.uBT_WW, PV}, {BU.FA_EE, PUs}, {BV.FA_EE, PVs},
                         {BU.FA_E0, PUs}, {BV.FA_E0, PVs}, {BU.FA_W0, PUs}, {BV.FA_W0, PVs}, {BU.FA_WW, PUs}, {BV.FA_WW, PVs}})) return rc;
      btcl_derive(hs);
    } else {
      btcl_derive(0);
    }
    if (apply_OBCs && early_btcl_pass) { if (int rc = setup_specified()) return rc; }
  } else if (nonlin_cont) {
    face_areas_eta(s, 1);
  } else {
    const double Z_to_H = g.Z_to_H, Zr = cs->Z_ref;
    launch2d(s, is - 2, ie + 1, js - 1, je + 1, [=] __device__(int I, int j) {
      const double H1 = (g.bathyT[g.h2(I, j)] + Zr) * Z_to_H, H2 = (g.bathyT[g.h2(I + 1, j)] + Zr) * Z_to_H;
      double D = 0.0;
      if ((H1 > 0.0) && (H2 > 0.0)) D = g.dy_Cu[g.u2(I, j)] * (2.0 * H1 * H2) / (H1 + H2);
      w.Datu[g.u2(I, j)] = D;
    });
    launch2d(s, is - 1, ie + 1, js - 2, je + 1, [=] __device__(int i, int J) {
      const double H1 = (g.bathyT[g.h2(i, J)] + Zr) * Z_to_H, H2 = (g.bathyT[g.h2(i, J + 1)] + Zr) * Z_to_H;
      double D = 0.0;
      if ((H1 > 0.0) && (H2 > 0.0)) D = g.dx_Cv[g.v2(i, J)] * (2.0 * H1 * H2) / (H1 + H2);
      w.Datv[g.v2(i, J)] = D;
    });
  }

  hipLaunchKernelGGL(bt_pre_face_kernel<0>, grid2d(is - 1, ie, js, je), dim3(64, 4), 0, s, g, w, p, c.frhatu, dvru, dUc, dpb, duh0, duu0,
                     dU, dbu, dtx, dtbx, c.IDatu);
  hipLaunchKernelGGL(bt_pre_face_kernel<1>, grid2d(is, ie, js - 1, je), dim3(64, 4), 0, s, g, w, p, c.frhatv, dvrv, dVc, dpb, dvh0, dvv0,
                     dV, dbv, dty, dtby, c.IDatv);

  if (apply_OBCs) {
    for (int n = 0; n < obc->number_of_segments; n++) {
      const mom6hip_obc_segment_t &S = obc->segment[n];
      if (!S.on_pe) continue;
      const int I = S.IsdB, J = S.JsdB, Isq = is - 1, Ieq = ie, Jsq = js - 1, Jeq = je;
      const int dirn = S.direction;
      if (S.is_N_or_S && (J >= Jsq - 1) && (J <= Jeq + 1)) {
        M6_REQUIRE(J >= g.jsd && J + 1 <= g.jed && S.isd >= g.isd && S.ied <= g.ied, "btstep: OBC segment %d lies outside the data domain", n + 1);
        launch2d(s, std::max(Isq - 1, S.isd), std::min(Ieq + 2, S.ied), J, J, [=] __device__(int i, int j) {
          if (dirn == MOM6HIP_OBC_DIRECTION_N) w.gtot_S[g.h2(i, j + 1)] = w.gtot_S[g.h2(i, j)];
          else w.gtot_N[g.h2(i, j)] = w.gtot_N[g.h2(i, j + 1)];
        });
      } else if (S.is_E_or_W && (I >= Isq - 1) && (I <= Ieq + 1)) {
        M6_REQUIRE(I >= g.isd && I + 1 <= g.ied && S.jsd >= g.jsd && S.jed <= g.jed, "btstep: OBC segment %d lies outside the data domain", n + 1);
        launch2d(s, I, I, std::max(Jsq - 1, S.jsd), std::min(Jeq + 2, S.jed), [=] __device__(int i, int j) {
          if (dirn == MOM6HIP_OBC_DIRECTION_E) w.gtot_W[g.h2(i + 1, j)] = w.gtot_W[g.h2(i, j)];
          else w.gtot_E[g.h2(i, j)] = w.gtot_E[g.h2(i + 1, j)];
        });
      }
    }
    M6_HIP(hipMemcpyAsync(w.ubt_first, w.ubt, sz.u2, hipMemcpyDeviceToDevice, s));
    M6_HIP(hipMemcpyAsync(w.vbt_first, w.vbt, sz.v2, hipMemcpyDeviceToDevice, s));
  }

  if (add_uh0) {
    if (use_BT_cont && cs->adjust_BT_cont) {
      if (int rc = pass({{w.ubt0, PU}, {w.vbt0, PV}, {w.uhbtS, PU}, {w.vhbtS, PV}})) return rc;
      for (int dir = 0; dir < 2; dir++) {
        const Btcl B = dir ? w.BV : w.BU;
        const double *ubt = dir ? w.vbt0 : w.ubt0, *uhbt = dir ? w.vhbtS : w.uhbtS;
        launch2d(s, (dir ? is : is - 1) - hs, ie + hs, (dir ? js - 1 : js) - hs, je + hs, [=] __device__(int i, int j) {
          const long n = dir ? g.v2(i, j) : g.u2(i, j);
          const double ub = ubt[n], uh = uhbt[n], dtl = 1.0;
          if ((dtl * ub > B.uBT_WW[n]) && (dtl * uh > B.uh_WW[n])) {
            B.uBT_WW[n] = dtl * ub;
            if (3.0 * uh < 2.0 * ub * B.FA_W0[n]) {
              B.uh_crvW[n] = (uh - ub * B.FA_W0[n]) / ((dtl * dtl) * ((ub * ub) * ub));
            } else {
              B.FA_W0[n] = 1.5 * uh / ub;
              B.uh_crvW[n] = -0.5 * uh / ((dtl * dtl) * ((ub * ub) * ub));
            }
            B.uh_WW[n] = dtl * uh;
          } else if ((dtl * ub < B.uBT_EE[n]) && (dtl * uh < B.uh_EE[n])) {
            B.uBT_EE[n] = dtl * ub;
            if (3.0 * uh < 2.0 * ub * B.FA_E0[n]) {
              B.uh_crvE[n] = (uh - ub * B.FA_E0[n]) / ((dtl * dtl) * ((ub * ub) * ub));
            } else {
              B.FA_E0[n] = 1.5 * uh / ub;
              B.uh_crvE[n] = -0.5 * uh / ((dtl * dtl) * ((ub * ub) * ub));
            }
            B.uh_EE[n] = dtl * uh;
          }
        });
      }
    }
    launch2d(s, is - 1, ie, js, je, [=] __device__(int I, int j) {
      const long n = g.u2(I, j);
      w.uhbt0[n] = w.uhbtS[n] - (use_BT_cont ? find_uhbt(w.ubt0[n], w.BU, n) : w.Datu[n] * w.ubt0[n]);
    });
    launch2d(s, is, ie, js - 1, je, [=] __device__(int i, int J) {
      const long n = g.v2(i, J);
      w.vhbt0[n] = w.vhbtS[n] - (use_BT_cont ? find_uhbt(w.vbt0[n], w.BV, n) : w.Datv[n] * w.vbt0[n]);
    });
    if (apply_u_OBCs) launch2d(s, is - 1, ie, js, je, [=] __device__(int I, int j) { if (w.obc_u[g.u2(I, j)]) w.uhbt0[g.u2(I, j)] = 0.0; });
    if (apply_v_OBCs) launch2d(s, is, ie, js - 1, je, [=] __device__(int i, int J) { if (w.obc_v[g.v2(i, J)]) w.vhbt0[g.v2(i, J)] = 0.0; });
  }

  {
    const int sad = cs->Sadourny;
    launch2d(s, isvf - 1, ievf + 1, jsvf - 1, jevf, [=] __device__(int i, int j) {
      const double q00 = w.q[g.q2(i, j)], qm0 = w.q[g.q2(i - 1, j)];
      if (sad) {
        w.amer[g.u2(i - 1, j)] = w.DCor_u[g.u2(i - 1, j)] * qm0;
        w.bmer[g.u2(i, j)] = w.DCor_u[g.u2(i, j)] * q00;
        w.cmer[g.u2(i, j + 1)] = w.DCor_u[g.u2(i, j + 1)] * q00;
        w.dmer[g.u2(i - 1, j + 1)] = w.DCor_u[g.u2(i - 1, j + 1)] * qm0;
      } else {
        const double qmm = w.q[g.q2(i - 1, j - 1)], q0m = w.q[g.q2(i, j - 1)], q0p = w.q[g.q2(i, j + 1)], qmp = w.q[g.q2(i - 1, j + 1)];
        w.amer[g.u2(i - 1, j)] = w.DCor_u[g.u2(i - 1, j)] * ((q00 + qmm) + qm0) / 3.0;
        w.bmer[g.u2(i, j)] = w.DCor_u[g.u2(i, j)] * (q00 + (qm0 + q0m)) / 3.0;
        w.cmer[g.u2(i, j + 1)] = w.DCor_u[g.u2(i, j + 1)] * (q00 + (qm0 + q0p)) / 3.0;
        w.dmer[g.u2(i - 1, j + 1)] = w.DCor_u[g.u2(i - 1, j + 1)] * ((q00 + qmp) + qm0) / 3.0;
// ... 248 lines not shown
    if (e0 == hipSuccess) {
      if (with_passes) rc = run_loop(ctx->cap_stream, n0, n1);
      else { run_steps(ctx->cap_stream, n0, n1); rc = 0; }
    }
    hipGraph_t graph = nullptr;
    hipError_t e1 = (e0 == hipSuccess) ? hipStreamEndCapture(ctx->cap_stream, &graph) : e0;
    ctx->stream = saved;
    M6_REQUIRE(rc == 0 && e1 == hipSuccess && graph, "btstep: capturing the barotropic subcycle as a hipGraph failed (%s)",
               hipGetErrorString(e1));
    { size_t nn = 0; if (hipGraphGetNodes(graph, nullptr, &nn) == hipSuccess) ctx->bt_graph_nodes_last = (long)nn; }
    hipGraphExec_t exec = nullptr;
    hipError_t e2 = hipGraphInstantiate(&exec, graph, nullptr, nullptr, 0);
    (void)hipGraphDestroy(graph);
    M6_REQUIRE(e2 == hipSuccess && exec, "btstep: hipGraphInstantiate failed (%s)", hipGetErrorString(e2));
    if (ctx->bt_graphs.size() >= 256) {
      (void)hipGraphExecDestroy((hipGraphExec_t)ctx->bt_graphs.front().second);
      ctx->bt_graphs.erase(ctx->bt_graphs.begin());
    }
    ctx->bt_graphs.push_back({key, (void *)exec});
    ctx->bt_graph_captures++;
    *out = exec;
    return 0;
  };
  static const bool graph_off = getenv("MOM6HIP_BT_GRAPH") && atoi(getenv("MOM6HIP_BT_GRAPH")) == 0;
  if (graph_off) {
    if (int rc = run_loop(s, 1, nt)) return rc;
  } else if (m6::multi_tile(ctx) && [&] {
               int nseg = 0;
               for (int n = 1; n <= nt; n++) if (n == 1 || rng[n].pass_first) nseg++;
               return nseg > 100;
             }()) {
    if (int rc = run_loop(s, 1, nt)) return rc;
  } else if (m6::multi_tile(ctx)) {
    int n0 = 1;
    while (n0 <= nt) {
      int n1 = n0;
      while (n1 + 1 <= nt && !rng[n1 + 1].pass_first) n1++;
      if (rng[n0].pass_first) { if (int rc = do_pass(n0)) return rc; }
      hipGraphExec_t exec = nullptr;
      if (int rc = graph_of(n0, n1, false, &exec)) return rc;
      M6_HIP(hipGraphLaunch(exec, s));
      ctx->bt_graph_launches++;
      n0 = n1 + 1;
    }
  } else {
    hipGraphExec_t exec = nullptr;
    if (int rc = graph_of(1, nt, true, &exec)) return rc;
    m6::KTimer kt(ctx, MOM6HIP_KT_BT_SUBCYCLE);
    M6_HIP(hipGraphLaunch(exec, s));
    ctx->bt_graph_launches++;
  }
  M6_HIP(hipGetLastError());
  if (fused && nt % 2 == 1) {
    M6_HIP(hipMemcpyAsync(w.eta, alt_eta, sz.h2, hipMemcpyDeviceToDevice, s));
    M6_HIP(hipMemcpyAsync(w.ubt, alt_ubt, sz.u2, hipMemcpyDeviceToDevice, s));
    M6_HIP(hipMemcpyAsync(w.vbt, alt_vbt, sz.v2, hipMemcpyDeviceToDevice, s));
    M6_HIP(hipMemcpyAsync(w.uhbtp, alt_uhbtp, sz.u2, hipMemcpyDeviceToDevice, s));
    M6_HIP(hipMemcpyAsync(w.vhbtp, alt_vhbtp, sz.v2, hipMemcpyDeviceToDevice, s));
  }

  {
    const double dgeo_de = p.dgeo_de;
    launch2d(s, is, ie, js, je, [=] __device__(int i, int j) {
      const long n = g.h2(i, j);
      double ea;
      if (interp) ea = dgeo_de * (0.5 * (w.eta[n] + deta_in[n]) - (w.eta_PF_1[n] + 0.5 * w.d_eta_PF[n]));
      else ea = dgeo_de * (0.5 * (w.eta[n] + deta_in[n]) - w.eta_PF[n]);
      w.e_anom[n] = ea;
      if (find_etaav) detaav[n] = w.eta_sum[n] * 1.0;
      deta_out[n] = w.eta_wtd[n] * 1.0;
    });
    for (int d = 0; d < 2 && apply_OBCs; d++) {
      if (!(d ? apply_v_OBCs : apply_u_OBCs)) continue;
      const int32_t *code = d ? w.obc_v : w.obc_u;
      launch2d(s, d ? is : is - 1, ie, d ? js - 1 : js, je, [=] __device__(int i, int j) {
        const int cde = code[d ? g.v2(i, j) : g.u2(i, j)];
        const long c0 = g.h2(i, j), c1 = d ? g.h2(i, j + 1) : g.h2(i + 1, j);
        if (cde & OB_PLUS) w.e_anom[c1] = w.e_anom[c0];
        else if (cde & OB_MINUS) w.e_anom[c0] = w.e_anom[c1];
      });
    }
    if (find_etaav) { if (int rc = pass({{detaav, PH}, {w.e_anom, PH}, {c.ubtav, PU}, {c.vbtav, PV}, {duhbtav, PU}, {dvhbtav, PV}})) return rc; }
    else { if (int rc = pass({{w.e_anom, PH}, {c.ubtav, PU}, {c.vbtav, PV}, {duhbtav, PU}, {dvhbtav, PV}})) return rc; }
    hipLaunchKernelGGL(bt_accel_layer_kernel<0>, grid2d(is - 1, ie, js, je), dim3(64, 4), 0, s, g, w, dpb, dalu, accel_underflow);
    hipLaunchKernelGGL(bt_accel_layer_kernel<1>, grid2d(is, ie, js - 1, je), dim3(64, 4), 0, s, g, w, dpb, dalv, accel_underflow);
    for (int d = 0; d < 2 && apply_OBCs; d++) {
      if (!(d ? apply_v_OBCs : apply_u_OBCs)) continue;
      const int32_t *code = d ? w.obc_v : w.obc_u;
      const double *wtd = d ? w.vbt_wtd : w.ubt_wtd, *first = d ? w.vbt_first : w.ubt_first;
      double *accel = d ? dalv : dalu;
      const long fstr = d ? (long)g.nih * (g.njh + 1) : (long)(g.nih + 1) * g.njh;
      const int nk = g.nk;
      launch2d(s, d ? is : is - 1, ie, d ? js - 1 : js, je, [=] __device__(int i, int j) {
        const long f = d ? g.v2(i, j) : g.u2(i, j);
        if (!code[f]) return;
        const double a = (wtd[f] - first[f]) / dt;
        for (int k = 0; k < nk; k++) accel[f + fstr * k] = a;
      });
    }
  }
  M6_HIP(hipGetLastError());
  return st.finish();
}

}
```

### mom6_amd/csrc/common.hpp

```cpp
#pragma once

#include <hip/hip_runtime.h>
#include <cstdint>
#include <cstdio>
#include <cstring>
#include <functional>
#include <string>
#include <utility>
#include <vector>

#include "../../include/mom6hip.h"

struct mom6hip_ctx;
struct m6_native_domain;

namespace m6 {

void set_error(const char *fmt, ...);
struct ErrorKeeper {
  ErrorKeeper();
  ~ErrorKeeper();
  char saved[1024];
};

#define M6_HIP(call)                                                                        \
  do {                                                                                      \
    hipError_t e_ = (call);                                                                 \
    if (e_ != hipSuccess) {                                                                 \
      m6::set_error("%s:%d: %s failed: %s", __FILE__, __LINE__, #call, hipGetErrorString(e_)); \
      return 1;                                                                             \
    }                                                                                       \
  } while (0)

#define M6_REQUIRE(cond, ...)            \
  do {                                   \
    if (!(cond)) {                       \
      m6::set_error(__VA_ARGS__);        \
      return 2;                          \
    }                                    \
  } while (0)

struct GridDev {
  int isc, iec, jsc, jec, isd, ied, jsd, jed, nk;
  int nih, njh;
  int tripolar_n;
  double Angstrom_H, H_subroundoff, dZ_subroundoff, H_to_Z, Z_to_H, g_Earth, Rho0;
  const double *mask2dT, *areaT, *IareaT, *dxT, *dyT, *IdxT, *IdyT, *bathyT;
  const double *mask2dCu, *dxCu, *dyCu, *dy_Cu, *IdxCu, *IdyCu, *areaCu, *IareaCu;
  const double *mask2dCv, *dxCv, *dyCv, *dx_Cv, *IdxCv, *IdyCv, *areaCv, *IareaCv;
  const double *mask2dBu, *dxBu, *dyBu, *areaBu, *IareaBu, *CoriolisBu, *IdxBu, *IdyBu;
  const double *uh_neglect, *vh_neglect;
  __host__ __device__ inline long h2(int i, int j) const { return (long)(i - isd) + (long)nih * (j - jsd); }
  __host__ __device__ inline long u2(int I, int j) const { return (long)(I - isd + 1) + (long)(nih + 1) * (j - jsd); }
  __host__ __device__ inline long v2(int i, int J) const { return (long)(i - isd) + (long)nih * (J - jsd + 1); }
  __host__ __device__ inline long q2(int I, int J) const { return (long)(I - isd + 1) + (long)(nih + 1) * (J - jsd + 1); }
  __host__ __device__ inline long h3(int i, int j, int k) const { return h2(i, j) + (long)nih * njh * k; }
  __host__ __device__ inline long u3(int I, int j, int k) const { return u2(I, j) + (long)(nih + 1) * njh * k; }
  __host__ __device__ inline long v3(int i, int J, int k) const { return v2(i, J) + (long)nih * (njh + 1) * k; }
  __host__ __device__ inline long nh3() const { return (long)nih * njh * nk; }
  __host__ __device__ inline long nu3() const { return (long)(nih + 1) * njh * nk; }
  __host__ __device__ inline long nv3() const { return (long)nih * (njh + 1) * nk; }
};

__device__ __forceinline__ double min2(double a, double b) { return a < b ? a : b; }
__device__ __forceinline__ double max2(double a, double b) { return a > b ? a : b; }

struct DevBuf {
  void *p = nullptr;
  size_t bytes = 0;
  int reserve(size_t n);
  void release();
};

struct HostTable {
  DevBuf buf;
  std::vector<double> last;
  const double *get(const double *host, size_t n);
};
enum { TABLE_PGF_RLAY = 0, TABLE_PGF_GPRIME, TABLE_SVML_RLAY, TABLE_TD_RLAY, TABLE_TD_GPRIME, TABLE_COUNT = 8 };

}

struct mom6hip_ctx {
  mom6hip_grid_t host;
  m6::GridDev g;
  hipStream_t stream = nullptr;
  std::vector<void *> metric_allocs;
  double *d_metric[64] = {};

  m6::DevBuf hprev, uhr, vhr, flags, stage[16], tr_stage[64];
  m6::DevBuf pool[64];
  m6::DevBuf rk2_scratch;
  m6::DevBuf rk2_eta_PF_start;
  int rk2_scratch_layout = 0;
  m6::DevBuf hv_pack;
  bool hv_pack_ready = false;
  m6::DevBuf hv_str;
  m6::DevBuf cont_hmid;
  uint64_t overlap[4] = {0, 0, 0, 0};
  uint64_t pgf_face_launches[2] = {0, 0};
  int cont_phase = 0;
  struct BcAccelFuse { const double *au, *av, *diffu, *diffv; double *u_bc, *v_bc; int inviscid; bool done; };
  BcAccelFuse *bc_fuse = nullptr;
  bool cont_fluxes_only = false;
  m6::DevBuf sv_rlay;
  m6::DevBuf adv_gen;
  m6::DevBuf adv_obc[64];
  int adv_obc_n = 0;
  m6::HostTable tables[m6::TABLE_COUNT];
  uint64_t xfer[4] = {0, 0, 0, 0};
  m6::DevBuf ale_sub;
  m6::DevBuf ale_side;
  std::vector<const void *> lds_configured;
  struct ObcTable { int site; uint64_t key; m6::DevBuf buf; size_t bytes; uint64_t last_use; std::vector<char> host; };
  std::vector<ObcTable> obc_tables;
  uint64_t obc_table_clock = 0, obc_table_builds = 0;
  m6::DevBuf vv_ntrunc;
  bool vv_ntrunc_ready = false;
  m6::DevBuf vv_kvml[2];
  const void *vv_kvml_h = nullptr;
  std::vector<std::pair<std::string, void *>> bt_graphs;
  hipStream_t cap_stream = nullptr;
  static constexpr int NSIDE = 4;
  hipStream_t side_stream[NSIDE] = {nullptr, nullptr, nullptr, nullptr};
  hipEvent_t side_fork = nullptr, side_join[NSIDE] = {nullptr, nullptr, nullptr, nullptr};
  long bt_graph_captures = 0, bt_graph_launches = 0, bt_graph_nodes_last = 0;
  int *h_domore_k = nullptr;
  m6_native_domain *native = nullptr;
  mom6hip_halo_fn halo_cb = nullptr;
  mom6hip_sum_fn sum_cb = nullptr;
  bool cb_stream_ordered = false;
  mom6hip_min_fn min_cb = nullptr;
  void *min_user = nullptr;
  void *cb_user = nullptr;
  int num_PEs = 0;
  bool poison_passes = false;
  bool split_rows_always = false;
  int poison_now = 0;
  struct PendingPass { std::vector<double *> f; std::vector<int32_t> pos, nk; } pending;
  m6::DevBuf efp_acc;
  std::vector<double> DL_depth, DL_area, DL_vol_below;
  std::vector<int> DL_lH;
  struct StageSlot { m6::DevBuf buf; hipEvent_t snap = nullptr, done = nullptr; };
  std::vector<StageSlot> stage_slots;
  int stage_next = 0;
  hipStream_t copy_stream = nullptr;
  bool ktiming = false;
  std::vector<std::pair<hipEvent_t, hipEvent_t>> kt_events[MOM6HIP_KT_SLOTS];
  bool timing = false;
  mom6hip_advect_timing_t adv_timing = {};
};

namespace m6 {

struct KTimer {
  mom6hip_ctx *c; int slot; hipEvent_t e0 = nullptr, e1 = nullptr;
  KTimer(mom6hip_ctx *ctx, int s) : c(ctx), slot(s) {
    if (!c->ktiming) return;
    if (hipEventCreate(&e0) != hipSuccess || hipEventCreate(&e1) != hipSuccess) { e0 = e1 = nullptr; return; }
    (void)hipEventRecord(e0, c->stream);
  }
  ~KTimer() {
    if (!e0) return;
    (void)hipEventRecord(e1, c->stream);
    c->kt_events[slot].push_back({e0, e1});
  }
};

int group_pass(mom6hip_ctx *ctx, double *const *fields, const int32_t *pos, const int32_t *nk, int n);
int start_group_pass(mom6hip_ctx *ctx, double *const *fields, const int32_t *pos, const int32_t *nk, int n);
int complete_group_pass(mom6hip_ctx *ctx);
bool pass_leaves_x_final(mom6hip_ctx *ctx);
void row_window(mom6hip_ctx *ctx, int j0, int j1);
void row_window_reset(mom6hip_ctx *ctx);
int halo_wrap_dir(mom6hip_ctx *ctx, double *f, int pos, int nk, int dir, hipStream_t stream);
int halo_fold_north(mom6hip_ctx *ctx, double *f, int pos_flags, int nk, hipStream_t stream);
int halo_pack_on(mom6hip_ctx *ctx, double *const *fields, const int32_t *pos, const int32_t *nk_each, const int32_t *a0, int32_t nfields,
                 int32_t dir, int32_t width, double *buf, int32_t pack, int64_t *count, hipStream_t stream);
int native_start_group_pass(mom6hip_ctx *ctx, double *const *fields, const int32_t *pos, const int32_t *nk, int n);
int native_complete_group_pass(mom6hip_ctx *ctx);
bool native_x_is_local(mom6hip_ctx *ctx);
void native_pass_sides(mom6hip_ctx *ctx, int sides[2]);
int native_allreduce(mom6hip_ctx *ctx, void *values, int n, bool is_int_sum);
int native_allreduce_dev(mom6hip_ctx *ctx, void *dvalues, int n, int kind, void *host_copy);
int sum_across_PEs_dev(mom6hip_ctx *ctx, int32_t *dvalues, int n, int32_t *host_copy);
int min_across_PEs_dev_u64(mom6hip_ctx *ctx, unsigned long long *dvalues, int n, unsigned long long *host_copy);
void native_domain_destroy(mom6hip_ctx *ctx);
// ... 59 lines not shown
```

### mom6_amd/csrc/dyn_split_rk2.hip

```cpp
#include "common.hpp"

#include <cstdlib>
#include <initializer_list>
#include <utility>

namespace m6 {

}

namespace {

template <class F> __global__ void __launch_bounds__(256) range3d_kernel(int i0, int i1, int j0, int j1, F f) {
  const int i = i0 + blockIdx.x * 64 + threadIdx.x, j = j0 + blockIdx.y * 4 + threadIdx.y;
  if (i <= i1 && j <= j1) f(i, j, (int)blockIdx.z);
}
template <class F> void launch3d(hipStream_t st, int i0, int i1, int j0, int j1, int nk, F f) {
  if (i1 < i0 || j1 < j0) return;
  dim3 grid((i1 - i0 + 64) / 64, (j1 - j0 + 4) / 4, nk), block(64, 4);
  hipLaunchKernelGGL(range3d_kernel<F>, grid, block, 0, st, i0, i1, j0, j1, f);
}

struct Sz { size_t h2, h3, u3, v3; };
Sz sizes(const m6::GridDev &g) {
  Sz s;
// ... 345 lines not shown
  double *vp = (double *)(blk + 3 * sz.u3), *v_bc = (double *)(blk + 3 * sz.u3 + sz.v3), *vh_in = (double *)(blk + 3 * sz.u3 + 2 * sz.v3);
  double *hp = (double *)(blk + 3 * sz.u3 + 3 * sz.v3), *eta_pred = (double *)(blk + 3 * sz.u3 + 3 * sz.v3 + sz.h3);
  double *u_av = cs->u_av, *v_av = cs->v_av, *h_av = cs->h_av, *eta = cs->eta;

  if (fresh) M6_HIP(hipMemsetAsync(blk, 0, blk_bytes, s));
  static const bool hp_whole = getenv("MOM6HIP_HP_COPY_WHOLE") && atoi(getenv("MOM6HIP_HP_COPY_WHOLE")) == 1;
  if (hp_whole) {
    M6_HIP(hipMemcpyAsync(hp, h, sz.h3, hipMemcpyDeviceToDevice, s));
  } else {
    auto copy_rect = [&](int i0, int i1, int j0, int j1) {
      launch3d(s, i0, i1, j0, j1, nz, [=] __device__(int i, int j, int k) { hp[g.h3(i, j, k)] = h[g.h3(i, j, k)]; });
    };
    copy_rect(g.isd, g.ied, g.jsd, js - 1); copy_rect(g.isd, g.ied, je + 1, g.jed);
    copy_rect(g.isd, is - 1, js, je); copy_rect(ie + 1, g.ied, js, je);
  }

  const bool inviscid = (cs->hooks == nullptr) && (cs->hor_visc == nullptr);
  const bool vv_fused = VV && !(hk && (hk->visc_remnant_pred || hk->vertvisc));
  const bool need_up1 = (!inviscid || VV) && !vv_fused;
  const bool kv_once = vv_fused && kvml_once();
  const m6::KvmlProfile kv_first = kv_once ? m6::KVML_PRODUCE : m6::KVML_AS_NOW, kv_later = kv_once ? m6::KVML_CONSUME : m6::KVML_AS_NOW;
  mom6hip_ctx::BcAccelFuse fuse1{nullptr, nullptr, cs->diffu, cs->diffv, u_bc, v_bc, inviscid ? 1 : 0, false};
  static const bool fuse_off = getenv("MOM6HIP_BC_FUSE") && atoi(getenv("MOM6HIP_BC_FUSE")) == 0;
  const bool try_fuse1 = !need_up1 && !fuse_off;
  if (try_fuse1 && cs->CAu_pred_stored) { fuse1.au = cs->CAu_pred; fuse1.av = cs->CAv_pred; ctx->bc_fuse = &fuse1; }
  const int rc_pf = mom6hip_pressureforce_fv_bouss(ctx, cs->PressureForce_CSp, cs->eqn_of_state, h, T, S, step_p_surf(cs), cs->PFu, cs->PFv,
                                                   cs->pbce, cs->eta_PF, D);
  ctx->bc_fuse = nullptr;
  if (rc_pf) return rc_pf;
  double *eta_PF_start = nullptr;
  CALL(step_eta_PF_start(ctx, cs, &eta_PF_start));
  if (!cs->CAu_pred_stored) {
    if (try_fuse1) { fuse1.au = cs->PFu; fuse1.av = cs->PFv; ctx->bc_fuse = &fuse1; }
    const int rc_ca = mom6hip_coradcalc(ctx, cs->CoriolisAdv, u_av, v_av, h_av, uh, vh, cs->CAu_pred, cs->CAv_pred, D);
    ctx->bc_fuse = nullptr;
    if (rc_ca) return rc_ca;
  }

  auto bc_accel = [&](const double *CAu, const double *CAv, bool first_up) {
    const double *PFu = cs->PFu, *PFv = cs->PFv, *diffu = cs->diffu, *diffv = cs->diffv;
    const bool need_up = first_up && (!inviscid || VV) && !vv_fused;
    launch3d(s, Isq, Ieq, js, je, nz, [=] __device__(int I, int j, int k) {
      const long n = g.u3(I, j, k);
      double a = (CAu[n] + PFu[n]);
      if (inviscid) a = (a == 0.0) ? 0.0 : a; else a = a + diffu[n];
      u_bc[n] = a;
      if (need_up) up[n] = g.mask2dCu[g.u2(I, j)] * (u_inst[n] + dt * a);
    });
    launch3d(s, is, ie, Jsq, Jeq, nz, [=] __device__(int i, int J, int k) {
      const long n = g.v3(i, J, k);
      double a = (CAv[n] + PFv[n]);
      if (inviscid) a = (a == 0.0) ? 0.0 : a; else a = a + diffv[n];
      v_bc[n] = a;
      if (need_up) vp[n] = g.mask2dCv[g.v2(i, J)] * (v_inst[n] + dt * a);
    });
  };
  if (!fuse1.done) bc_accel(cs->CAu_pred, cs->CAv_pred, true);
  if (hk && hk->visc_remnant_pred) {
    M6_HIP(hipStreamSynchronize(s));
    M6_REQUIRE(hk->visc_remnant_pred(hk->user, up, vp, h, dt, cs->visc_rem_u, cs->visc_rem_v) == 0, "visc_remnant_pred hook failed");
  } else if (VV) {
    if (cs->set_visc_CSp && cs->set_visc_CSp->dynamic_viscous_ML) {
      M6_REQUIRE(cs->visc->ustar && cs->visc->nkml_visc_u && cs->visc->nkml_visc_v,
                 "step_MOM_dyn_split_RK2: DYNAMIC_VISCOUS_ML needs forces%%ustar (visc->ustar) and visc%%nkml_visc_u / nkml_visc_v");
      CALL(m6::set_viscous_ML_dev(ctx, cs->set_visc_CSp, u_inst, v_inst, h, T, S, cs->eqn_of_state, taux, tauy, cs->visc->ustar,
                                  (double *)cs->visc->nkml_visc_u, (double *)cs->visc->nkml_visc_v, dt));
    }
    const m6::VelIncrement inc1{u_inst, v_inst, u_bc, v_bc, nullptr, nullptr, dt};
    CALL(m6::vertvisc_step_inc(ctx, VV, up, vp, h, nullptr, nullptr, nullptr, cs->visc, dt, 0, nullptr, nullptr, cs->visc_rem_u, cs->visc_rem_v,
                               vv_fused ? &inc1 : nullptr, D, kv_first));
  }
  CALL(pass_start(ctx, {{eta, PH | P2D}, {cs->visc_rem_u, PUs}, {cs->visc_rem_v, PVs}}, nz, 0));

  if (!BT_cont_BT_thick) CALL(mom6hip_btcalc(ctx, BT, h, nullptr, nullptr, 0, D));
  CALL(mom6hip_bt_mass_source(ctx, BT, h, eta, 1, D));
  if (BTC || cs->BT_use_layer_fluxes) {
    ctx->cont_fluxes_only = true;
    const int rc_c = continuity_around_pass(ctx, [&]() -> int {
      return mom6hip_continuity(ctx, cs->continuity_CSp, u_inst, v_inst, h, hp, uh_in, vh_in, dt, nullptr, nullptr, cs->visc_rem_u,
                                cs->visc_rem_v, nullptr, nullptr, BTC, nullptr, nullptr, D);
    });
    ctx->cont_fluxes_only = false;
    if (rc_c) return rc_c;
    if (BT_cont_BT_thick) CALL(mom6hip_btcalc(ctx, BT, h, BTC->h_u, BTC->h_v, 0, D));
  } else {
    CALL(m6::complete_group_pass(ctx));
  }
  if (calc_dtbt) CALL(mom6hip_set_dtbt_eta(ctx, BT, eta, cs->pbce, nullptr, 0.0, 0.0, D));
  const bool lf = cs->BT_use_layer_fluxes != 0;
  CALL(mom6hip_btstep(ctx, BT, u_inst, v_inst, eta, dt, u_bc, v_bc, taux, tauy, RZ_to_H, cs->pbce, cs->eta_PF, u_av, v_av,
                      cs->u_accel_bt, cs->v_accel_bt, eta_pred, cs->uhbt, cs->vhbt, cs->visc_rem_u, cs->visc_rem_v, BTC, eta_PF_start, nullptr,
                      nullptr, lf ? uh_in : nullptr, lf ? vh_in : nullptr, lf ? u_inst : nullptr, lf ? v_inst : nullptr, nullptr, D));

  const double dt_pred = dt * cs->be;
  if (!vv_fused) {
    const double *abu = cs->u_accel_bt, *abv = cs->v_accel_bt;
    launch3d(s, is, ie, Jsq, Jeq, nz, [=] __device__(int i, int J, int k) {
      const long n = g.v3(i, J, k);
      vp[n] = g.mask2dCv[g.v2(i, J)] * (v_inst[n] + dt_pred * (v_bc[n] + abv[n]));
    });
    launch3d(s, Isq, Ieq, js, je, nz, [=] __device__(int I, int j, int k) {
      const long n = g.u3(I, j, k);
      up[n] = g.mask2dCu[g.u2(I, j)] * (u_inst[n] + dt_pred * (u_bc[n] + abu[n]));
    });
  }
  if (hk && hk->vertvisc) {
    M6_HIP(hipStreamSynchronize(s));
    M6_REQUIRE(hk->vertvisc(hk->user, up, vp, h, dt_pred, cs->visc_rem_u, cs->visc_rem_v) == 0, "vertvisc hook failed");
  } else if (VV) {
    const m6::VelIncrement inc2{u_inst, v_inst, u_bc, v_bc, cs->u_accel_bt, cs->v_accel_bt, dt_pred};
    CALL(m6::vertvisc_step_inc(ctx, VV, up, vp, h, nullptr, taux, tauy, cs->visc, dt_pred, 1, nullptr, nullptr, cs->visc_rem_u, cs->visc_rem_v,
                               vv_fused ? &inc2 : nullptr, D, kv_later));
  }
  CALL(pass_start(ctx, {{cs->visc_rem_u, PUs}, {cs->visc_rem_v, PVs}, {up, PU}, {vp, PV}}, nz, 1));
  CALL(continuity_around_pass(ctx, [&]() -> int {
    return mom6hip_continuity(ctx, cs->continuity_CSp, up, vp, h, hp, uh, vh, dt, cs->uhbt, cs->vhbt, cs->visc_rem_u, cs->visc_rem_v,
                              u_av, v_av, BTC, nullptr, nullptr, D);
  }));
  const bool hv_hook = !cs->hor_visc && hk && hk->horizontal_viscosity;
  auto after_hp_uv = [&]() -> int {
    const m6::GridDev w = ctx->g;
    launch3d(s, is - 2, ie + 2, w.jsc - 2, w.jec + 2, nz, [=] __device__(int i, int j, int k) {
      const long n = g.h3(i, j, k);
      h_av[n] = 0.5 * (h[n] + hp[n]);
    });
    if (cs->hor_visc) {
      if (m6::horizontal_viscosity_dev(ctx, cs->hor_visc, u_av, v_av, h_av, cs->diffu, cs->diffv, BTC ? BTC->h_u : nullptr,
                                       BTC ? BTC->h_v : nullptr)) return 1;
    }
    if (!hv_hook) CALL(mom6hip_coradcalc(ctx, cs->CoriolisAdv, u_av, v_av, h_av, uh, vh, cs->CAu, cs->CAv, D));
    return 0;
  };
  CALL(pass_start(ctx, {{hp, PH}, {u_av, PU}, {v_av, PV}, {uh, PU}, {vh, PV}}, nz, 2));
  CALL(mom6hip_bt_mass_source(ctx, BT, hp, eta_pred, 0, D));
  if (BT_cont_BT_thick) CALL(mom6hip_btcalc(ctx, BT, h, BTC->h_u, BTC->h_v, 0, D));
  mom6hip_ctx::BcAccelFuse fuse2{cs->PFu, cs->PFv, cs->diffu, cs->diffv, u_bc, v_bc, inviscid ? 1 : 0, false};
  if (!fuse_off) ctx->bc_fuse = &fuse2;
  int rc_ap = around_pass(ctx, after_hp_uv);
  if (rc_ap == 0 && hv_hook) {
    rc_ap = hipStreamSynchronize(s) == hipSuccess ? 0 : 1;
    if (rc_ap == 0 && hk->horizontal_viscosity(hk->user, u_av, v_av, h_av, cs->diffu, cs->diffv) != 0) {
      m6::set_error("horizontal_viscosity hook failed"); rc_ap = 1;
    }
    if (rc_ap == 0) rc_ap = mom6hip_coradcalc(ctx, cs->CoriolisAdv, u_av, v_av, h_av, uh, vh, cs->CAu, cs->CAv, D);
  }
  ctx->bc_fuse = nullptr;
  if (rc_ap) return rc_ap;
  if (!fuse2.done) bc_accel(cs->CAu, cs->CAv, false);
  CALL(mom6hip_btstep(ctx, BT, u_inst, v_inst, eta, dt, u_bc, v_bc, taux, tauy, RZ_to_H, cs->pbce, cs->eta_PF, u_av, v_av,
                      cs->u_accel_bt, cs->v_accel_bt, eta_pred, cs->uhbt, cs->vhbt, cs->visc_rem_u, cs->visc_rem_v, BTC, eta_PF_start, nullptr,
                      nullptr, lf ? uh : nullptr, lf ? vh : nullptr, lf ? u_av : nullptr, lf ? v_av : nullptr, eta_av, D));
  launch3d(s, is, ie, js, je, 1, [=] __device__(int i, int j, int) { eta[g.h2(i, j)] = eta_pred[g.h2(i, j)]; });
  if (!vv_fused) {
    const double *abu = cs->u_accel_bt, *abv = cs->v_accel_bt;
    launch3d(s, Isq, Ieq, js, je, nz, [=] __device__(int I, int j, int k) {
      const long n = g.u3(I, j, k);
      u_inst[n] = g.mask2dCu[g.u2(I, j)] * (u_inst[n] + dt * (u_bc[n] + abu[n]));
    });
    launch3d(s, is, ie, Jsq, Jeq, nz, [=] __device__(int i, int J, int k) {
      const long n = g.v3(i, J, k);
      v_inst[n] = g.mask2dCv[g.v2(i, J)] * (v_inst[n] + dt * (v_bc[n] + abv[n]));
    });
  }
  if (hk && hk->vertvisc) {
    M6_HIP(hipStreamSynchronize(s));
    M6_REQUIRE(hk->vertvisc(hk->user, u_inst, v_inst, h, dt, cs->visc_rem_u, cs->visc_rem_v) == 0, "vertvisc hook failed");
  } else if (VV) {
    const m6::VelIncrement inc3{u_inst, v_inst, u_bc, v_bc, cs->u_accel_bt, cs->v_accel_bt, dt};
    CALL(m6::vertvisc_step_inc(ctx, VV, u_inst, v_inst, h, nullptr, taux, tauy, cs->visc, dt, 1, nullptr, nullptr, cs->visc_rem_u, cs->visc_rem_v,
                               vv_fused ? &inc3 : nullptr, D, kv_later));
  }
  launch3d(s, is - 2, ie + 2, js - 2, je + 2, nz, [=] __device__(int i, int j, int k) { h_av[g.h3(i, j, k)] = h[g.h3(i, j, k)]; });
  CALL(pass_start(ctx, {{cs->visc_rem_u, PUs}, {cs->visc_rem_v, PVs}, {u_inst, PU}, {v_inst, PV}}, nz, 3));
  CALL(continuity_around_pass(ctx, [&]() -> int {
    return mom6hip_continuity(ctx, cs->continuity_CSp, u_inst, v_inst, h, h, uh, vh, dt, cs->uhbt, cs->vhbt, cs->visc_rem_u,
                              cs->visc_rem_v, u_av, v_av, nullptr, nullptr, nullptr, D);
  }));
  auto accumulate = [&](int ja, int jb, int Ja, int Jb) {
    launch3d(s, is - 2, ie + 2, ja, jb, nz, [=] __device__(int i, int j, int k) {
      const long n = g.h3(i, j, k);
      h_av[n] = 0.5 * (h_av[n] + h[n]);
    });
    launch3d(s, Isq - 2, Ieq + 2, ja, jb, nz, [=] __device__(int I, int j, int k) {
      const long n = g.u3(I, j, k);
      uhtr[n] = uhtr[n] + uh[n] * dt;
    });
    launch3d(s, is - 2, ie + 2, Ja, Jb, nz, [=] __device__(int i, int J, int k) {
      const long n = g.v3(i, J, k);
      vhtr[n] = vhtr[n] + vh[n] * dt;
    });
  };
  auto next_CA = [&]() -> int {
    if (cs->store_CAu) CALL(mom6hip_coradcalc(ctx, cs->CoriolisAdv, u_av, v_av, h_av, uh, vh, cs->CAu_pred, cs->CAv_pred, D));
    return 0;
  };
  CALL(pass_start(ctx, {{h, PH}, {u_av, PU}, {v_av, PV}, {uh, PU}, {vh, PV}}, nz, 4));
  if (split_rows(ctx)) {
    ctx->overlap[0]++;
    const int W = is - g.isd;
    accumulate(js + 2, je - 2, Jsq + 2, Jeq - 2);
    m6::row_window(ctx, js + W + 2, je - W - 2);
    int rc = next_CA();
    m6::row_window_reset(ctx);
    if (rc) { m6::ErrorKeeper keep; m6::complete_group_pass(ctx); return rc; }
    CALL(m6::complete_group_pass(ctx));
    accumulate(js - 2, js + 1, Jsq - 2, Jsq + 1);
    accumulate(je - 1, je + 2, Jeq - 1, Jeq + 2);
    m6::row_window(ctx, js, js + W + 1);
    rc = next_CA();
    if (!rc) { m6::row_window(ctx, je - W - 1, je); rc = next_CA(); }
    m6::row_window_reset(ctx);
    if (rc) return rc;
  } else {
    ctx->overlap[2]++;
    CALL(m6::complete_group_pass(ctx));
    accumulate(js - 2, je + 2, Jsq - 2, Jeq + 2);
    CALL(next_CA());
  }
  cs->CAu_pred_stored = cs->store_CAu ? 1 : 0;
  M6_HIP(hipGetLastError());
  return 0;
}


int mom6hip_dyn_split_rk2b_init(mom6hip_ctx_t *ctx, mom6hip_dyn_split_rk2_cs_t *cs, const double *h) {
  M6_REQUIRE(ctx && h, "dyn_split_rk2b_init: null argument");
  CALL(check(cs, "dyn_split_rk2b_init"));
  M6_REQUIRE(cs->du_av_inst && cs->dv_av_inst, "dyn_split_rk2b_init: du_av_inst / dv_av_inst are not allocated");
  const m6::GridDev g = ctx->g;
  const Sz sz = sizes(g);
  hipStream_t s = ctx->stream;
  {
    double *eta = cs->eta;
    const double Z_to_H = g.Z_to_H;
    const long hstr = (long)g.nih * g.njh;
    const int nz = g.nk;
    launch3d(s, g.isc, g.iec, g.jsc, g.jec, 1, [=] __device__(int i, int j, int) {
      const long n = g.h2(i, j);
      double e = -Z_to_H * g.bathyT[n];
      for (int k = 0; k < nz; k++) e = e + h[n + hstr * k];
      eta[n] = e;
    });
  }
  M6_HIP(hipMemsetAsync(cs->diffu, 0, sz.u3, s)); M6_HIP(hipMemsetAsync(cs->diffv, 0, sz.v3, s));
  M6_HIP(hipMemsetAsync(cs->du_av_inst, 0, sz.u3 / g.nk, s)); M6_HIP(hipMemsetAsync(cs->dv_av_inst, 0, sz.v3 / g.nk, s));
  M6_HIP(hipMemsetAsync(cs->u_av, 0, sz.u3, s)); M6_HIP(hipMemsetAsync(cs->v_av, 0, sz.v3, s));
  {
    double *vru = cs->visc_rem_u, *vrv = cs->visc_rem_v;
    launch3d(s, g.isd - 1, g.ied, g.jsd, g.jed, g.nk, [=] __device__(int i, int j, int k) { vru[g.u3(i, j, k)] = 1.0; });
    launch3d(s, g.isd, g.ied, g.jsd - 1, g.jed, g.nk, [=] __device__(int i, int j, int k) { vrv[g.v3(i, j, k)] = 1.0; });
  }
  M6_HIP(hipGetLastError());
  return 0;
}

int mom6hip_step_dyn_split_rk2b(mom6hip_ctx_t *ctx, mom6hip_dyn_split_rk2_cs_t *cs, double *u_av, double *v_av, double *h,
                                const double *T, const double *S, double dt, const double *taux, const double *tauy, double RZ_to_H,
                                double *uh, double *vh, double *uhtr, double *vhtr, double *eta_av, int32_t calc_dtbt) {
  M6_REQUIRE(ctx && u_av && v_av && h && taux && tauy && uh && vh && uhtr && vhtr && eta_av, "step_MOM_dyn_split_RK2b: null argument");
  CALL(check(cs, "step_MOM_dyn_split_RK2b"));
  M6_REQUIRE(!cs->eqn_of_state || (T && S), "step_MOM_dyn_split_RK2b: an equation of state needs tv%%T and tv%%S");
  M6_REQUIRE(cs->du_av_inst && cs->dv_av_inst, "step_MOM_dyn_split_RK2b: du_av_inst / dv_av_inst are not allocated");
  const mom6hip_obc_t *OBC = cs->OBC;
  M6_REQUIRE(!OBC || !cs->hooks, "step_MOM_dyn_split_RK2b: host-side parameterisations (hooks) are not provided with an associated OBC");
  static const bool obc_one_tile = getenv("MOM6HIP_OBC_ONE_TILE") && atoi(getenv("MOM6HIP_OBC_ONE_TILE")) == 1;
  M6_REQUIRE(!OBC || !obc_one_tile || !m6::multi_tile(ctx), "step_MOM_dyn_split_RK2b: an associated OBC is provided on one tile (MOM6HIP_OBC_ONE_TILE)");
  const m6::GridDev g = ctx->g;
  const Sz sz = sizes(g);
  hipStream_t s = ctx->stream;
  const int D = MOM6HIP_MEM_DEVICE;
  const int is = g.isc, ie = g.iec, js = g.jsc, je = g.jec, nz = g.nk;
  const int Isq = is - 1, Ieq = ie, Jsq = js - 1, Jeq = je;
  mom6hip_barotropic_cs_t *BT = cs->barotropic_CSp;
  const mom6hip_bt_cont_t *BTC = cs->BT_cont;
  const bool BT_cont_BT_thick = BTC && BTC->h_u && BTC->h_v;
  const mom6hip_visc_hooks_t *hk = cs->hooks;
  mom6hip_vertvisc_cs_t *VV = cs->vertvisc_CSp;
  M6_REQUIRE(!VV || cs->visc, "step_MOM_dyn_split_RK2b: vertvisc_CSp needs the visc argument (cs->visc)");

  const size_t blk_bytes = 3 * sz.u3 + 3 * sz.v3 + sz.h3 + sz.h2 + (OBC ? sz.u3 + sz.v3 : 0);
  const bool fresh = ctx->rk2_scratch.bytes < blk_bytes || ctx->rk2_scratch_layout != 2;
  M6_REQUIRE(ctx->rk2_scratch.reserve(blk_bytes) == 0, "step_MOM_dyn_split_RK2b: out of device memory");
  ctx->rk2_scratch_layout = 2;
  char *blk = (char *)ctx->rk2_scratch.p;
  double *up = (double *)blk, *u_bc = (double *)(blk + sz.u3), *uh_in = (double *)(blk + 2 * sz.u3);
  double *vp = (double *)(blk + 3 * sz.u3), *v_bc = (double *)(blk + 3 * sz.u3 + sz.v3), *vh_in = (double *)(blk + 3 * sz.u3 + 2 * sz.v3);
  double *hp = (double *)(blk + 3 * sz.u3 + 3 * sz.v3), *eta_pred = (double *)(blk + 3 * sz.u3 + 3 * sz.v3 + sz.h3);
  double *u_inst = cs->u_av, *v_inst = cs->v_av, *h_av = cs->h_av, *eta = cs->eta;
  if (fresh) M6_HIP(hipMemsetAsync(blk, 0, blk_bytes, s));
  M6_HIP(hipMemcpyAsync(hp, h, sz.h3, hipMemcpyDeviceToDevice, s));
  double *u_old = nullptr, *v_old = nullptr;
  if (OBC) {
    u_old = (double *)(blk + 3 * sz.u3 + 3 * sz.v3 + sz.h3 + sz.h2); v_old = (double *)((char *)u_old + sz.u3);
    M6_HIP(hipMemcpyAsync(u_old, u_av, sz.u3, hipMemcpyDeviceToDevice, s));
    M6_HIP(hipMemcpyAsync(v_old, v_av, sz.v3, hipMemcpyDeviceToDevice, s));
  }
  auto coradcalc = [&](double *CAu, double *CAv) -> int {
    return OBC ? mom6hip_coradcalc_obc(ctx, cs->CoriolisAdv, OBC, u_av, v_av, cs->h_av, uh, vh, CAu, CAv, D)
               : mom6hip_coradcalc(ctx, cs->CoriolisAdv, u_av, v_av, cs->h_av, uh, vh, CAu, CAv, D);
  };
  auto btcalc = [&](const double *hu, const double *hv) -> int {
    return OBC ? mom6hip_btcalc_obc(ctx, BT, h, hu, hv, 0, OBC, D) : mom6hip_btcalc(ctx, BT, h, hu, hv, 0, D);
  };
  const bool kv_once = VV && !OBC && !(hk && (hk->visc_remnant_pred || hk->vertvisc)) && kvml_once();
  auto vertvisc_step = [&](double *uu, double *vv, double dtx, int update) -> int {
    if (!OBC) return m6::vertvisc_step_inc(ctx, VV, uu, vv, h, nullptr, update ? taux : nullptr, update ? tauy : nullptr, cs->visc, dtx, update, nullptr,
                                           nullptr, cs->visc_rem_u, cs->visc_rem_v, nullptr, D,
                                           !kv_once ? m6::KVML_AS_NOW : (update ? m6::KVML_CONSUME : m6::KVML_PRODUCE));
    CALL(mom6hip_vertvisc_coef_obc(ctx, VV, uu, vv, h, nullptr, cs->visc, dtx, OBC, D));
    if (update) CALL(mom6hip_vertvisc_obc(ctx, VV, uu, vv, h, taux, tauy, cs->visc, dtx, nullptr, nullptr, OBC, D));
    return mom6hip_vertvisc_remnant(ctx, VV, cs->visc, cs->visc_rem_u, cs->visc_rem_v, dtx, D);
  };

  CALL(mom6hip_continuity_obc(ctx, cs->continuity_CSp, OBC, u_av, v_av, h, hp, uh, vh, dt, nullptr, nullptr, nullptr, nullptr, nullptr, nullptr,
                              nullptr, nullptr, nullptr, D));
  CALL(mom6hip_pressureforce_fv_bouss(ctx, cs->PressureForce_CSp, cs->eqn_of_state, h, T, S, step_p_surf(cs), cs->PFu, cs->PFv, cs->pbce,
                                      cs->eta_PF, D));
  double *eta_PF_start = nullptr;
  CALL(step_eta_PF_start(ctx, cs, &eta_PF_start));
  CALL(pass(ctx, {{hp, PH}, {uh, PU}, {vh, PV}}, nz));
  auto set_h_av = [&]() {
    launch3d(s, is - 2, ie + 2, js - 2, je + 2, nz, [=] __device__(int i, int j, int k) {
      const long n = g.h3(i, j, k);
      h_av[n] = 0.5 * (h[n] + hp[n]);
    });
  };
  set_h_av();
  auto hor_visc = [&]() -> int {
    if (cs->hor_visc && OBC) {
      CALL(mom6hip_horizontal_viscosity_obc(ctx, cs->hor_visc, u_av, v_av, h_av, cs->diffu, cs->diffv, dt, BTC ? BTC->h_u : nullptr,
                                            BTC ? BTC->h_v : nullptr, OBC, D));
    } else if (cs->hor_visc) {
      if (m6::horizontal_viscosity_dev(ctx, cs->hor_visc, u_av, v_av, h_av, cs->diffu, cs->diffv, BTC ? BTC->h_u : nullptr,
                                       BTC ? BTC->h_v : nullptr)) return 1;
    } else if (hk && hk->horizontal_viscosity) {
      M6_HIP(hipStreamSynchronize(s));
      M6_REQUIRE(hk->horizontal_viscosity(hk->user, u_av, v_av, h_av, cs->diffu, cs->diffv) == 0, "horizontal_viscosity hook failed");
    }
    return 0;
  };
  CALL(coradcalc(cs->CAu_pred, cs->CAv_pred));
  CALL(hor_visc());

  auto bc_accel = [&](const double *CAu, const double *CAv, bool first_up) {
    const double *PFu = cs->PFu, *PFv = cs->PFv, *diffu = cs->diffu, *diffv = cs->diffv;
    const bool need_up = first_up && (VV || (hk && hk->visc_remnant_pred)) && !OBC;
    launch3d(s, Isq, Ieq, js, je, nz, [=] __device__(int I, int j, int k) {
      const long n = g.u3(I, j, k);
      const double a = (CAu[n] + PFu[n]) + diffu[n];
      u_bc[n] = a;
      if (need_up) up[n] = g.mask2dCu[g.u2(I, j)] * (u_av[n] + dt * a);
    });
    launch3d(s, is, ie, Jsq, Jeq, nz, [=] __device__(int i, int J, int k) {
      const long n = g.v3(i, J, k);
      const double a = (CAv[n] + PFv[n]) + diffv[n];
      v_bc[n] = a;
      if (need_up) vp[n] = g.mask2dCv[g.v2(i, J)] * (v_av[n] + dt * a);
    });
  };
  bc_accel(cs->CAu_pred, cs->CAv_pred, true);
  if (OBC) {
    CALL(mom6hip_open_boundary_zero_normal_flow(ctx, OBC, u_bc, v_bc, D));
    if (VV) {
      launch3d(s, Isq, Ieq, js, je, nz, [=] __device__(int I, int j, int k) {
        const long n = g.u3(I, j, k);
        up[n] = g.mask2dCu[g.u2(I, j)] * (u_av[n] + dt * u_bc[n]);
      });
      launch3d(s, is, ie, Jsq, Jeq, nz, [=] __device__(int i, int J, int k) {
        const long n = g.v3(i, J, k);
        vp[n] = g.mask2dCv[g.v2(i, J)] * (v_av[n] + dt * v_bc[n]);
      });
    }
  }
  if (hk && hk->visc_remnant_pred) {
    M6_HIP(hipStreamSynchronize(s));
    M6_REQUIRE(hk->visc_remnant_pred(hk->user, up, vp, h, dt, cs->visc_rem_u, cs->visc_rem_v) == 0, "visc_remnant_pred hook failed");
  } else if (VV) {
    if (cs->set_visc_CSp && cs->set_visc_CSp->dynamic_viscous_ML) {
      M6_REQUIRE(cs->visc->ustar && cs->visc->nkml_visc_u && cs->visc->nkml_visc_v,
                 "step_MOM_dyn_split_RK2b: DYNAMIC_VISCOUS_ML needs forces%%ustar (visc->ustar) and visc%%nkml_visc_u / nkml_visc_v");
      CALL(m6::set_viscous_ML_dev(ctx, cs->set_visc_CSp, u_av, v_av, h, T, S, cs->eqn_of_state, taux, tauy, cs->visc->ustar,
                                  (double *)cs->visc->nkml_visc_u, (double *)cs->visc->nkml_visc_v, dt));
    }
    CALL(vertvisc_step(up, vp, dt, 0));
  }
// ... 109 lines not shown
```

Measured before the change: 27.15.

## Defer btcalc frhat computation into btstep pre-face kernel and merge accel-layer kernels

Adds a deferred btcalc path that records h_u/h_v and, if the next btstep uses the same control structure, computes the frhat fractions inside the pre-face kernel. This removes the separate btcalc_given launches and their extra pass over the layer data. Any other entry point (init, set_dtbt, btcalc_obc, or a mismatched btstep) flushes the pending work first, which adds state tracking across calls. Separately, the u and v accel-layer kernels are merged into one launch that shares the pbce and e_anom loads, at the cost of some divergence at the domain edges.

After: 27.25 (median of 6 runs). Within noise of the previous version (+0.4%).

```diff
diff --git a/include/mom6hip.h b/include/mom6hip.h
--- a/include/mom6hip.h
+++ b/include/mom6hip.h
@@ -444,6 +444,9 @@
 int mom6hip_btcalc_obc(mom6hip_ctx_t *ctx, mom6hip_barotropic_cs_t *cs, const double *h, const double *h_u, const double *h_v,
                        int32_t may_use_default, const struct mom6hip_obc *obc, int32_t memspace);
 
+int mom6hip_btcalc_defer(mom6hip_ctx_t *ctx, mom6hip_barotropic_cs_t *cs, const double *h, const double *h_u, const double *h_v,
+                         int32_t memspace);
+
 int mom6hip_bt_mass_source(mom6hip_ctx_t *ctx, mom6hip_barotropic_cs_t *cs, const double *h, const double *eta,
                            int32_t set_cor, int32_t memspace);
 
diff --git a/mom6_amd/_lib.py b/mom6_amd/_lib.py
--- a/mom6_amd/_lib.py
+++ b/mom6_amd/_lib.py
@@ -13,7 +13,7 @@
     "mom6hip_sync", "mom6hip_malloc", "mom6hip_free", "mom6hip_sync_to_device",
     "mom6hip_sync_to_host", "mom6hip_halo_update", "mom6hip_advect_tracer", "mom6hip_set_timing",
     "mom6hip_advect_get_timing", "mom6hip_ale_remap_tracers", "mom6hip_ale_plm_edge_values", "mom6hip_coradcalc", "mom6hip_continuity", "mom6hip_pressureforce_fv_bouss", "mom6hip_pressureforce_fv_nonbouss", "mom6hip_pgf_face_launches", "mom6hip_calculate_density", "mom6hip_set_domain_callbacks",
-    "mom6hip_barotropic_init", "mom6hip_btcalc", "mom6hip_bt_mass_source", "mom6hip_set_dtbt", "mom6hip_memset_zero", "mom6hip_transfer_stats", "mom6hip_debug_poison_passes", "mom6hip_tracer_hordiff_varmix", "mom6hip_tracer_hordiff_neutral", "mom6hip_tracer_hordiff_epipycnal", "mom6hip_continuity_obc", "mom6hip_coradcalc_obc", "mom6hip_vertvisc_coef_obc", "mom6hip_update_segment_tracer_reservoirs", "mom6hip_advect_tracer_obc", "mom6hip_btstep_obc", "mom6hip_horizontal_viscosity_obc", "mom6hip_set_viscous_bbl_obc", "mom6hip_btcalc_obc", "mom6hip_vertvisc_obc", "mom6hip_radiation_open_bdry_conds", "mom6hip_open_boundary_zero_normal_flow", "mom6hip_overlap_stats", "mom6hip_thickness_diffuse", "mom6hip_mixedlayer_restrat", "mom6hip_mixedlayer_restrat_mu", "mom6hip_start_group_pass", "mom6hip_complete_group_pass", "mom6hip_set_dtbt_eta", "mom6hip_btstep",
+    "mom6hip_barotropic_init", "mom6hip_btcalc", "mom6hip_btcalc_defer", "mom6hip_bt_mass_source", "mom6hip_set_dtbt", "mom6hip_memset_zero", "mom6hip_transfer_stats", "mom6hip_debug_poison_passes", "mom6hip_tracer_hordiff_varmix", "mom6hip_tracer_hordiff_neutral", "mom6hip_tracer_hordiff_epipycnal", "mom6hip_continuity_obc", "mom6hip_coradcalc_obc", "mom6hip_vertvisc_coef_obc", "mom6hip_update_segment_tracer_reservoirs", "mom6hip_advect_tracer_obc", "mom6hip_btstep_obc", "mom6hip_horizontal_viscosity_obc", "mom6hip_set_viscous_bbl_obc", "mom6hip_btcalc_obc", "mom6hip_vertvisc_obc", "mom6hip_radiation_open_bdry_conds", "mom6hip_open_boundary_zero_normal_flow", "mom6hip_overlap_stats", "mom6hip_thickness_diffuse", "mom6hip_mixedlayer_restrat", "mom6hip_mixedlayer_restrat_mu", "mom6hip_start_group_pass", "mom6hip_complete_group_pass", "mom6hip_set_dtbt_eta", "mom6hip_btstep",
     "mom6hip_dyn_split_rk2_init", "mom6hip_step_dyn_split_rk2", "mom6hip_dyn_split_rk2b_init", "mom6hip_step_dyn_split_rk2b",
     "mom6hip_ale_regrid", "mom6hip_ale_remap_set_h_vel", "mom6hip_ale_remap_set_h_vel_via_dz", "mom6hip_ale_remap_velocities", "mom6hip_halo_pack", "mom6hip_set_min_callback", "mom6hip_kernel_timing", "mom6hip_set_callback_stream_ordered", "mom6hip_bt_graph_stats", "mom6hip_bt_graph_nodes",
     "mom6hip_vertvisc_coef", "mom6hip_vertvisc", "mom6hip_vertvisc_remnant", "mom6hip_vertvisc_ntrunc", "mom6hip_vertvisc_and_remnant", "mom6hip_vertvisc_step",
diff --git a/mom6_amd/barotropic.py b/mom6_amd/barotropic.py
--- a/mom6_amd/barotropic.py
+++ b/mom6_amd/barotropic.py
@@ -100,6 +100,7 @@
         cs = C.POINTER(_abi.BarotropicCS)
         L.mom6hip_barotropic_init.argtypes = [C.c_void_p, cs, C.c_int32]
         L.mom6hip_btcalc.argtypes = [C.c_void_p, cs, C.c_void_p, C.c_void_p, C.c_void_p, C.c_int32, C.c_int32]
+        L.mom6hip_btcalc_defer.argtypes = [C.c_void_p, cs, C.c_void_p, C.c_void_p, C.c_void_p, C.c_int32]
         L.mom6hip_btcalc_obc.argtypes = [C.c_void_p, cs, C.c_void_p, C.c_void_p, C.c_void_p, C.c_int32, C.POINTER(_abi.Obc), C.c_int32]
         L.mom6hip_bt_mass_source.argtypes = [C.c_void_p, cs, C.c_void_p, C.c_void_p, C.c_int32, C.c_int32]
         L.mom6hip_set_dtbt.argtypes = [C.c_void_p, cs, C.c_void_p, C.POINTER(_abi.BTCont), C.c_double, C.c_double, C.c_int32]
@@ -140,6 +141,14 @@
                                           _one_space(sp, CS, "btcalc")), "btcalc")
         return
     check(_setup().mom6hip_btcalc(G.handle, C.byref(CS.st), *args, int(bool(may_use_default)), _one_space(sp, CS, "btcalc")), "btcalc")
+
+
+def btcalc_defer(h, G: DeviceGrid, CS: barotropic_CS, h_u, h_v):
+    if not CS.module_is_initialized:
+        raise Mom6HipError("btcalc: Module MOM_barotropic must be initialized before it is used.")
+    sp = set()
+    args = [_P(sp, h), _P(sp, h_u), _P(sp, h_v)]
+    check(_setup().mom6hip_btcalc_defer(G.handle, C.byref(CS.st), *args, _one_space(sp, CS, "btcalc")), "btcalc")
 
 
 def bt_mass_source(h, eta, set_cor, G: DeviceGrid, CS: barotropic_CS):
diff --git a/mom6_amd/csrc/barotropic.hip b/mom6_amd/csrc/barotropic.hip
--- a/mom6_amd/csrc/barotropic.hip
+++ b/mom6_amd/csrc/barotropic.hip
@@ -110,9 +110,55 @@
   int nstep, use_BT_cont, interp_eta_PF, add_uh0, strong_drag, visc_rem_u_uh0, find_etaav, have_bot;
 };
 
-template <int DIR>
+struct PreFaceSums { double vel_cor = 0.0, gt_m = 0.0, gt_p = 0.0, uhS = 0.0, u0 = 0.0, ub = 0.0, av_rem = 0.0, force = 0.0; };
+__device__ __forceinline__ void pre_face_layer(PreFaceSums &a, const Par &p, double fr, double vr_in, double vcor, double pb_m, double pb_p,
+                                               const double *__restrict__ uh0, const double *__restrict__ u_uh0, long f3, double vin,
+                                               double bc) {
+  double vr = m6::min2(vr_in, 1.);
+  vr = m6::max2(vr, 1. - 0.5 * p.Instep / (vr + SUBROUNDOFF));
+  vr = m6::max2(vr, 0.);
+  const double wt = fr * vr;
+  a.vel_cor = a.vel_cor + wt * vcor;
+  a.gt_m = a.gt_m + pb_m * wt;
+  a.gt_p = a.gt_p + pb_p * wt;
+  if (p.add_uh0) {
+    a.uhS = a.uhS + uh0[f3];
+    a.u0 = a.u0 + (p.visc_rem_u_uh0 ? wt : fr) * u_uh0[f3];
+  }
+  a.ub = a.ub + wt * vin;
+  a.force = a.force + wt * bc;
+  a.av_rem = a.av_rem + fr * vr_in;
+}
+template <int DIR> __device__ __forceinline__ void pre_face_store(const Work &w, const Par &p, PreFaceSums a, double mask, long f2, long hm, long hp) {
+  if (fabs(a.ub) < p.vel_underflow) a.ub = 0.0;
+  double rem;
+  if (p.strong_drag) {
+    rem = mask * ((p.nstep * a.av_rem) / (1.0 + (p.nstep - 1) * a.av_rem));
+  } else {
+    rem = 0.0;
+    if (mask * a.av_rem > 0.0) rem = mask * cr_pow(a.av_rem, p.Instep);
+  }
+  if (DIR == 0) {
+    w.ubt_Cor[f2] = a.vel_cor; w.gtot_E[hm] = a.gt_m; w.gtot_W[hp] = a.gt_p; w.uhbtS[f2] = a.uhS; w.ubt0[f2] = a.u0;
+    w.ubt[f2] = a.ub; w.BT_force_u[f2] = a.force; w.bt_rem_u[f2] = rem;
+  } else {
+    w.vbt_Cor[f2] = a.vel_cor; w.gtot_N[hm] = a.gt_m; w.gtot_S[hp] = a.gt_p; w.vhbtS[f2] = a.uhS; w.vbt0[f2] = a.u0;
+    w.vbt[f2] = a.ub; w.BT_force_v[f2] = a.force; w.bt_rem_v[f2] = rem;
+  }
+}
+__device__ __forceinline__ double pre_face_force0(const Par &p, double mask, long f2, const double *__restrict__ tau,
+                                                  const double *__restrict__ tau_bot, const double *__restrict__ IDat,
+                                                  const double *__restrict__ visc_rem) {
+  if (!(mask > 0.0)) return 0.0;
+  double force = tau[f2] * p.RZ_to_H * IDat[f2] * visc_rem[f2];
+  if (p.have_bot) force = force - tau_bot[f2] * p.RZ_to_H * IDat[f2];
+  return force;
+}
+
+template <int DIR, int NKMAX>
 __global__ void __launch_bounds__(256)
-bt_pre_face_kernel(m6::GridDev g, Work w, Par p, const double *__restrict__ frhat, const double *__restrict__ visc_rem,
+bt_pre_face_kernel(m6::GridDev g, Work w, Par p, const double *__restrict__ frhat, const double *__restrict__ hw,
+                   double *__restrict__ frhat_out, double h_neglect, const double *__restrict__ visc_rem,
                    const double *__restrict__ vel_Cor, const double *__restrict__ pbce, const double *__restrict__ uh0,
                    const double *__restrict__ u_uh0, const double *__restrict__ vel_in, const double *__restrict__ bc_accel,
                    const double *__restrict__ tau, const double *__restrict__ tau_bot, const double *__restrict__ IDat) {
@@ -123,47 +169,50 @@
   const long fstr = DIR ? (long)g.nih * (g.njh + 1) : (long)(g.nih + 1) * g.njh;
   const long hm = g.h2(i, j), hp = DIR ? g.h2(i, j + 1) : g.h2(i + 1, j), hstr = (long)g.nih * g.njh;
   const double mask = DIR ? g.mask2dCv[f2] : g.mask2dCu[f2];
-
-  double vel_cor = 0.0, gt_m = 0.0, gt_p = 0.0, uhS = 0.0, u0 = 0.0, ub = 0.0, av_rem = 0.0, force;
-  if (mask > 0.0) {
-    force = tau[f2] * p.RZ_to_H * IDat[f2] * visc_rem[f2];
-    if (p.have_bot) force = force - tau_bot[f2] * p.RZ_to_H * IDat[f2];
+  const int nz = g.nk;
+
+  PreFaceSums a;
+  a.force = pre_face_force0(p, mask, f2, tau, tau_bot, IDat, visc_rem);
+  if constexpr (NKMAX == 0) {
+    for (int k = 0; k < nz; k++) {
+      const long f3 = f2 + fstr * k;
+      pre_face_layer(a, p, frhat[f3], visc_rem[f3], vel_Cor[f3], pbce[hm + hstr * k], pbce[hp + hstr * k], uh0, u_uh0, f3, vel_in[f3],
+                     bc_accel[f3]);
+    }
   } else {
-    force = 0.0;
-  }
-  for (int k = 0; k < g.nk; k++) {
-    const long f3 = f2 + fstr * k;
-    const double fr = frhat[f3], vr_in = visc_rem[f3];
-    double vr = m6::min2(vr_in, 1.);
-    vr = m6::max2(vr, 1. - 0.5 * p.Instep / (vr + SUBROUNDOFF));
-    vr = m6::max2(vr, 0.);
-    const double wt = fr * vr;
-    vel_cor = vel_cor + wt * vel_Cor[f3];
-    gt_m = gt_m + pbce[hm + hstr * k] * wt;
-    gt_p = gt_p + pbce[hp + hstr * k] * wt;
-    if (p.add_uh0) {
-      uhS = uhS + uh0[f3];
-      u0 = u0 + (p.visc_rem_u_uh0 ? wt : fr) * u_uh0[f3];
-    }
-    ub = ub + wt * vel_in[f3];
-    force = force + wt * bc_accel[f3];
-    av_rem = av_rem + fr * vr_in;
-  }
-  if (fabs(ub) < p.vel_underflow) ub = 0.0;
-  double rem;
-  if (p.strong_drag) {
-    rem = mask * ((p.nstep * av_rem) / (1.0 + (p.nstep - 1) * av_rem));
-  } else {
-    rem = 0.0;
-    if (mask * av_rem > 0.0) rem = mask * cr_pow(av_rem, p.Instep);
-  }
-  if (DIR == 0) {
-    w.ubt_Cor[f2] = vel_cor; w.gtot_E[hm] = gt_m; w.gtot_W[hp] = gt_p; w.uhbtS[f2] = uhS; w.ubt0[f2] = u0;
-    w.ubt[f2] = ub; w.BT_force_u[f2] = force; w.bt_rem_u[f2] = rem;
-  } else {
-    w.vbt_Cor[f2] = vel_cor; w.gtot_N[hm] = gt_m; w.gtot_S[hp] = gt_p; w.vhbtS[f2] = uhS; w.vbt0[f2] = u0;
-    w.vbt[f2] = ub; w.BT_force_v[f2] = force; w.bt_rem_v[f2] = rem;
-  }
+#ifdef BT_PRE_TWO_PASS
+    double tot = hw[f2];
+    for (int k = 1; k < nz; k++) tot = tot + hw[f2 + fstr * k];
+    const double Ihat = mask / (tot + h_neglect);
+    for (int k = 0; k < nz; k++) {
+      const long f3 = f2 + fstr * k;
+      const double fr = hw[f3] * Ihat;
+      frhat_out[f3] = fr;
+      pre_face_layer(a, p, fr, visc_rem[f3], vel_Cor[f3], pbce[hm + hstr * k], pbce[hp + hstr * k], uh0, u_uh0, f3, vel_in[f3],
+                     bc_accel[f3]);
+    }
+#else
+    double v[NKMAX];
+    const double *__restrict__ src = hw + f2;
+#pragma unroll
+    for (int k = 0; k < NKMAX; k++) { v[k] = (k < nz) ? *src : 0.0; src += fstr; }
+    double tot = v[0];
+#pragma unroll
+    for (int k = 1; k < NKMAX; k++) if (k < nz) tot = tot + v[k];
+    const double Ihat = mask / (tot + h_neglect);
+#pragma unroll
+    for (int k = 0; k < NKMAX; k++) {
+      if (k < nz) {
+        const long f3 = f2 + fstr * k;
+        const double fr = v[k] * Ihat;
+        frhat_out[f3] = fr;
+        pre_face_layer(a, p, fr, visc_rem[f3], vel_Cor[f3], pbce[hm + hstr * k], pbce[hp + hstr * k], uh0, u_uh0, f3, vel_in[f3],
+                       bc_accel[f3]);
+      }
+    }
+#endif
+  }
+  pre_face_store<DIR>(w, p, a, mask, f2, hm, hp);
 }
 
 template <int DIR, int NKMAX>
@@ -189,23 +238,31 @@
   for (int k = 0; k < NKMAX; k++) { if (k < nz) *dst = v[k] * Ihat; dst += fstr; }
 }
 
-template <int DIR>
 __global__ void __launch_bounds__(256)
-bt_accel_layer_kernel(m6::GridDev g, Work w, const double *__restrict__ pbce, double *__restrict__ accel, double accel_underflow) {
-  const int i = (DIR ? g.isc : g.isc - 1) + blockIdx.x * 64 + threadIdx.x;
-  const int j = (DIR ? g.jsc - 1 : g.jsc) + blockIdx.y * 4 + threadIdx.y;
+bt_accel_layer_kernel(m6::GridDev g, Work w, const double *__restrict__ pbce, double *__restrict__ accel_u, double *__restrict__ accel_v,
+                      double accel_underflow) {
+  const int i = g.isc - 1 + blockIdx.x * 64 + threadIdx.x, j = g.jsc - 1 + blockIdx.y * 4 + threadIdx.y;
   if (i > g.iec || j > g.jec) return;
-  const long f2 = DIR ? g.v2(i, j) : g.u2(i, j);
-  const long fstr = DIR ? (long)g.nih * (g.njh + 1) : (long)(g.nih + 1) * g.njh;
-  const long hm = g.h2(i, j), hp = DIR ? g.h2(i, j + 1) : g.h2(i + 1, j), hstr = (long)g.nih * g.njh;
-  const double abt = DIR ? w.v_accel_bt[f2] : w.u_accel_bt[f2];
-  const double gp = DIR ? w.gtot_S[hp] : w.gtot_W[hp], gm = DIR ? w.gtot_N[hm] : w.gtot_E[hm];
-  const double ep = w.e_anom[hp], em = w.e_anom[hm];
-  const double Id = DIR ? g.IdyCv[f2] : g.IdxCu[f2];
+  const bool do_u = j >= g.jsc, do_v = i >= g.isc;
+  if (!do_u && !do_v) return;
+  const long fu = g.u2(i, j), fv = g.v2(i, j), ustr = (long)(g.nih + 1) * g.njh, vstr = (long)g.nih * (g.njh + 1);
+  const long hc = g.h2(i, j), he = g.h2(i + 1, j), hn = g.h2(i, j + 1), hstr = (long)g.nih * g.njh;
+  const double ec = w.e_anom[hc];
+  double abt_u = 0.0, gW = 0.0, gE = 0.0, ee = 0.0, Idx = 0.0, abt_v = 0.0, gS = 0.0, gN = 0.0, en = 0.0, Idy = 0.0;
+  if (do_u) { abt_u = w.u_accel_bt[fu]; gW = w.gtot_W[he]; gE = w.gtot_E[hc]; ee = w.e_anom[he]; Idx = g.IdxCu[fu]; }
+  if (do_v) { abt_v = w.v_accel_bt[fv]; gS = w.gtot_S[hn]; gN = w.gtot_N[hc]; en = w.e_anom[hn]; Idy = g.IdyCv[fv]; }
   for (int k = 0; k < g.nk; k++) {
-    double a = (abt - ((pbce[hp + hstr * k] - gp) * ep - (pbce[hm + hstr * k] - gm) * em) * Id);
-    if (fabs(a) < accel_underflow) a = 0.0;
-    accel[f2 + fstr * k] = a;
+    const double pc = pbce[hc + hstr * k];
+    if (do_u) {
+      double a = (abt_u - ((pbce[he + hstr * k] - gW) * ee - (pc - gE) * ec) * Idx);
+      if (fabs(a) < accel_underflow) a = 0.0;
+      accel_u[fu + ustr * k] = a;
+    }
+    if (do_v) {
+      double a = (abt_v - ((pbce[hn + hstr * k] - gS) * en - (pc - gN) * ec) * Idy);
+      if (fabs(a) < accel_underflow) a = 0.0;
+      accel_v[fv + vstr * k] = a;
+    }
   }
 }
 
@@ -560,6 +617,39 @@
 
 dim3 grid2d(int i0, int i1, int j0, int j1) { return dim3((i1 - i0 + 64) / 64, (j1 - j0 + 4) / 4); }
 
+constexpr int BTCALC_GIVEN_NKMAX = 76;
+
+void launch_btcalc_given(mom6hip_ctx_t *ctx, int dir, const double *hw, double *fr) {
+  const m6::GridDev g = ctx->g;
+  const double h_neglect = g.H_subroundoff;
+  const dim3 grid = grid2d(dir ? g.isc : g.isc - 1, g.iec, dir ? g.jsc - 1 : g.jsc, g.jec), block(64, 4);
+  if (g.nk <= 32) {
+    if (dir) hipLaunchKernelGGL((btcalc_given_kernel<1, 32>), grid, block, 0, ctx->stream, g, hw, fr, h_neglect);
+    else hipLaunchKernelGGL((btcalc_given_kernel<0, 32>), grid, block, 0, ctx->stream, g, hw, fr, h_neglect);
+  } else {
+    if (dir) hipLaunchKernelGGL((btcalc_given_kernel<1, BTCALC_GIVEN_NKMAX>), grid, block, 0, ctx->stream, g, hw, fr, h_neglect);
+    else hipLaunchKernelGGL((btcalc_given_kernel<0, BTCALC_GIVEN_NKMAX>), grid, block, 0, ctx->stream, g, hw, fr, h_neglect);
+  }
+}
+
+int bt_given_flush(mom6hip_ctx_t *ctx) {
+  const mom6hip_ctx::BtGiven gv = ctx->bt_given;
+  if (!gv.cs) return 0;
+  ctx->bt_given = mom6hip_ctx::BtGiven();
+  launch_btcalc_given(ctx, 0, gv.h_u, gv.frhatu);
+  launch_btcalc_given(ctx, 1, gv.h_v, gv.frhatv);
+  M6_HIP(hipGetLastError());
+  return 0;
+}
+
+template <int DIR, class... A>
+void launch_pre_face(hipStream_t s, dim3 grid, const m6::GridDev &g, const Work &w, const Par &p, double *fr, const double *hw, A... rest) {
+  const double h_neglect = g.H_subroundoff;
+  if (!hw) hipLaunchKernelGGL((bt_pre_face_kernel<DIR, 0>), grid, dim3(64, 4), 0, s, g, w, p, (const double *)fr, hw, (double *)nullptr, h_neglect, rest...);
+  else if (g.nk <= 32) hipLaunchKernelGGL((bt_pre_face_kernel<DIR, 32>), grid, dim3(64, 4), 0, s, g, w, p, (const double *)nullptr, hw, fr, h_neglect, rest...);
+  else hipLaunchKernelGGL((bt_pre_face_kernel<DIR, BTCALC_GIVEN_NKMAX>), grid, dim3(64, 4), 0, s, g, w, p, (const double *)nullptr, hw, fr, h_neglect, rest...);
+}
+
 }
 
 extern "C" {
@@ -567,6 +657,7 @@
 int mom6hip_barotropic_init(mom6hip_ctx_t *ctx, mom6hip_barotropic_cs_t *cs, int32_t memspace) {
   M6_REQUIRE(ctx != nullptr, "barotropic_init: null context");
   if (int rc = check_cs(cs, "barotropic_init")) return rc;
+  if (int rc = bt_given_flush(ctx)) return rc;
   const m6::GridDev g = ctx->g;
   M6_REQUIRE(g.bathyT && g.areaT && g.mask2dT && g.mask2dCu && g.mask2dCv && g.CoriolisBu,
              "barotropic_init: bathyT, areaT, mask2dT, mask2dCu, mask2dCv and CoriolisBu are needed");
@@ -636,6 +727,7 @@
 int mom6hip_btcalc_obc(mom6hip_ctx_t *ctx, mom6hip_barotropic_cs_t *cs, const double *h, const double *h_u, const double *h_v,
                        int32_t may_use_default, const mom6hip_obc_t *obc, int32_t memspace) {
   M6_REQUIRE(ctx != nullptr && cs != nullptr && h != nullptr, "btcalc: null argument");
+  if (int rc = bt_given_flush(ctx)) return rc;
   const m6::GridDev g = ctx->g;
   const int sch = cs->hvel_scheme;
   int use_default = 0;
@@ -658,15 +750,8 @@
     const int32_t *side = side_d[dir];
     double *fr = dir ? frv : fru;
     const long fstr = dir ? (long)g.nih * (g.njh + 1) : (long)(g.nih + 1) * g.njh, hstr = (long)g.nih * g.njh;
-    if (hw && !side && g.nk <= 76) {
-      const dim3 grid = grid2d(dir ? g.isc : g.isc - 1, g.iec, dir ? g.jsc - 1 : g.jsc, g.jec), block(64, 4);
-      if (g.nk <= 32) {
-        if (dir) hipLaunchKernelGGL((btcalc_given_kernel<1, 32>), grid, block, 0, ctx->stream, g, hw, fr, h_neglect);
-        else hipLaunchKernelGGL((btcalc_given_kernel<0, 32>), grid, block, 0, ctx->stream, g, hw, fr, h_neglect);
-      } else {
-        if (dir) hipLaunchKernelGGL((btcalc_given_kernel<1, 76>), grid, block, 0, ctx->stream, g, hw, fr, h_neglect);
-        else hipLaunchKernelGGL((btcalc_given_kernel<0, 76>), grid, block, 0, ctx->stream, g, hw, fr, h_neglect);
-      }
+    if (hw && !side && g.nk <= BTCALC_GIVEN_NKMAX) {
+      launch_btcalc_given(ctx, dir, hw, fr);
       continue;
     }
     launch2d(ctx->stream, dir ? g.isc : g.isc - 1, g.iec, dir ? g.jsc - 1 : g.jsc, g.jec, [=] __device__(int i, int j) {
@@ -739,6 +824,17 @@
   return st.finish();
 }
 
+int mom6hip_btcalc_defer(mom6hip_ctx_t *ctx, mom6hip_barotropic_cs_t *cs, const double *h, const double *h_u, const double *h_v,
+                         int32_t memspace) {
+  M6_REQUIRE(ctx != nullptr && cs != nullptr && h != nullptr && h_u != nullptr && h_v != nullptr, "btcalc_defer: null argument");
+  M6_REQUIRE(cs->frhatu && cs->frhatv, "btcalc_defer: the control structure's state arrays must be allocated");
+  if (memspace != MOM6HIP_MEM_DEVICE || ctx->g.nk > BTCALC_GIVEN_NKMAX) return mom6hip_btcalc(ctx, cs, h, h_u, h_v, 0, memspace);
+  if (int rc = bt_given_flush(ctx)) return rc;
+  ctx->bt_given.cs = cs; ctx->bt_given.h_u = h_u; ctx->bt_given.h_v = h_v;
+  ctx->bt_given.frhatu = cs->frhatu; ctx->bt_given.frhatv = cs->frhatv;
+  return 0;
+}
+
 int mom6hip_bt_mass_source(mom6hip_ctx_t *ctx, mom6hip_barotropic_cs_t *cs, const double *h, const double *eta, int32_t set_cor,
                            int32_t memspace) {
   M6_REQUIRE(ctx != nullptr && cs != nullptr && h != nullptr && eta != nullptr, "bt_mass_source: null argument");
@@ -770,6 +866,7 @@
                          const mom6hip_bt_cont_t *BT_cont, double gtot_est, double SSH_add, int32_t memspace) {
   M6_REQUIRE(ctx != nullptr, "set_dtbt: null context");
   if (int rc = check_cs(cs, "set_dtbt")) return rc;
+  if (int rc = bt_given_flush(ctx)) return rc;
   const m6::GridDev g = ctx->g;
   const Sizes sz = sizes_of(g);
   m6::Stager st(ctx, memspace);
@@ -873,6 +970,14 @@
   M6_REQUIRE(g.bathyT && g.IareaT && g.areaT && g.IdxCu && g.IdyCv && g.dy_Cu && g.dx_Cv && g.mask2dT && g.mask2dCu &&
                  g.mask2dCv && g.CoriolisBu, "btstep: a metric array it needs was not given to grid_create");
   const int is = g.isc, ie = g.iec, js = g.jsc, je = g.jec;
+  const double *given_hu = nullptr, *given_hv = nullptr;
+  if (ctx->bt_given.cs == cs && ctx->bt_given.frhatu == cs->frhatu && ctx->bt_given.frhatv == cs->frhatv && !obc &&
+      memspace == MOM6HIP_MEM_DEVICE && g.nk <= BTCALC_GIVEN_NKMAX) {
+    given_hu = ctx->bt_given.h_u; given_hv = ctx->bt_given.h_v;
+    ctx->bt_given = mom6hip_ctx::BtGiven();
+  } else if (int rc = bt_given_flush(ctx)) {
+    return rc;
+  }
   const Sizes sz = sizes_of(g);
   const bool use_BT_cont = BT_cont != nullptr, interp = eta_PF_start != nullptr, add_uh0 = uh0 != nullptr;
   const bool find_etaav = etaav != nullptr, have_bot = taux_bot && tauy_bot;
@@ -1183,10 +1288,10 @@
     });
   }
 
-  hipLaunchKernelGGL(bt_pre_face_kernel<0>, grid2d(is - 1, ie, js, je), dim3(64, 4), 0, s, g, w, p, c.frhatu, dvru, dUc, dpb, duh0, duu0,
-                     dU, dbu, dtx, dtbx, c.IDatu);
-  hipLaunchKernelGGL(bt_pre_face_kernel<1>, grid2d(is, ie, js - 1, je), dim3(64, 4), 0, s, g, w, p, c.frhatv, dvrv, dVc, dpb, dvh0, dvv0,
-                     dV, dbv, dty, dtby, c.IDatv);
+  launch_pre_face<0>(s, grid2d(is - 1, ie, js, je), g, w, p, c.frhatu, given_hu, dvru, dUc, dpb, duh0, duu0, dU, dbu, dtx, dtbx,
+                     (const double *)c.IDatu);
+  launch_pre_face<1>(s, grid2d(is, ie, js - 1, je), g, w, p, c.frhatv, given_hv, dvrv, dVc, dpb, dvh0, dvv0, dV, dbv, dty, dtby,
+                     (const double *)c.IDatv);
 
   if (apply_OBCs) {
     for (int n = 0; n < obc->number_of_segments; n++) {
@@ -1601,8 +1706,7 @@
     }
     if (find_etaav) { if (int rc = pass({{detaav, PH}, {w.e_anom, PH}, {c.ubtav, PU}, {c.vbtav, PV}, {duhbtav, PU}, {dvhbtav, PV}})) return rc; }
     else { if (int rc = pass({{w.e_anom, PH}, {c.ubtav, PU}, {c.vbtav, PV}, {duhbtav, PU}, {dvhbtav, PV}})) return rc; }
-    hipLaunchKernelGGL(bt_accel_layer_kernel<0>, grid2d(is - 1, ie, js, je), dim3(64, 4), 0, s, g, w, dpb, dalu, accel_underflow);
-    hipLaunchKernelGGL(bt_accel_layer_kernel<1>, grid2d(is, ie, js - 1, je), dim3(64, 4), 0, s, g, w, dpb, dalv, accel_underflow);
+    hipLaunchKernelGGL(bt_accel_layer_kernel, grid2d(is - 1, ie, js - 1, je), dim3(64, 4), 0, s, g, w, dpb, dalu, dalv, accel_underflow);
     for (int d = 0; d < 2 && apply_OBCs; d++) {
       if (!(d ? apply_v_OBCs : apply_u_OBCs)) continue;
       const int32_t *code = d ? w.obc_v : w.obc_u;
diff --git a/mom6_amd/csrc/common.hpp b/mom6_amd/csrc/common.hpp
--- a/mom6_amd/csrc/common.hpp
+++ b/mom6_amd/csrc/common.hpp
@@ -103,6 +103,8 @@
   struct BcAccelFuse { const double *au, *av, *diffu, *diffv; double *u_bc, *v_bc; int inviscid; bool done; };
   BcAccelFuse *bc_fuse = nullptr;
   bool cont_fluxes_only = false;
+  struct BtGiven { const void *cs = nullptr; const double *h_u = nullptr, *h_v = nullptr; double *frhatu = nullptr, *frhatv = nullptr; };
+  BtGiven bt_given;
   m6::DevBuf sv_rlay;
   m6::DevBuf adv_gen;
   m6::DevBuf adv_obc[64];
diff --git a/mom6_amd/csrc/dyn_split_rk2.hip b/mom6_amd/csrc/dyn_split_rk2.hip
--- a/mom6_amd/csrc/dyn_split_rk2.hip
+++ b/mom6_amd/csrc/dyn_split_rk2.hip
@@ -451,7 +451,7 @@
     });
     ctx->cont_fluxes_only = false;
     if (rc_c) return rc_c;
-    if (BT_cont_BT_thick) CALL(mom6hip_btcalc(ctx, BT, h, BTC->h_u, BTC->h_v, 0, D));
+    if (BT_cont_BT_thick) CALL(mom6hip_btcalc_defer(ctx, BT, h, BTC->h_u, BTC->h_v, D));
   } else {
     CALL(m6::complete_group_pass(ctx));
   }
@@ -502,7 +502,7 @@
   };
   CALL(pass_start(ctx, {{hp, PH}, {u_av, PU}, {v_av, PV}, {uh, PU}, {vh, PV}}, nz, 2));
   CALL(mom6hip_bt_mass_source(ctx, BT, hp, eta_pred, 0, D));
-  if (BT_cont_BT_thick) CALL(mom6hip_btcalc(ctx, BT, h, BTC->h_u, BTC->h_v, 0, D));
+  if (BT_cont_BT_thick) CALL(mom6hip_btcalc_defer(ctx, BT, h, BTC->h_u, BTC->h_v, D));
   mom6hip_ctx::BcAccelFuse fuse2{cs->PFu, cs->PFv, cs->diffu, cs->diffv, u_bc, v_bc, inviscid ? 1 : 0, false};
   if (!fuse_off) ctx->bc_fuse = &fuse2;
   int rc_ap = around_pass(ctx, after_hp_uv);
@@ -669,7 +669,8 @@
                : mom6hip_coradcalc(ctx, cs->CoriolisAdv, u_av, v_av, cs->h_av, uh, vh, CAu, CAv, D);
   };
   auto btcalc = [&](const double *hu, const double *hv) -> int {
-    return OBC ? mom6hip_btcalc_obc(ctx, BT, h, hu, hv, 0, OBC, D) : mom6hip_btcalc(ctx, BT, h, hu, hv, 0, D);
+    if (OBC) return mom6hip_btcalc_obc(ctx, BT, h, hu, hv, 0, OBC, D);
+    return (hu && hv) ? mom6hip_btcalc_defer(ctx, BT, h, hu, hv, D) : mom6hip_btcalc(ctx, BT, h, hu, hv, 0, D);
   };
   const bool kv_once = VV && !OBC && !(hk && (hk->visc_remnant_pred || hk->vertvisc)) && kvml_once();
   auto vertvisc_step = [&](double *uu, double *vv, double dtx, int update) -> int {
```
